# goruck/semantic-segmentation-server

Measured on AMD Instinct MI355X. Metric: frames/sec (whole node) + p50 GetSegmentedObjects latency, 513x513 PASCAL VOC, higher is better.
Workload: dtype bf16; 1 GPU; model=DeepLabv3-MobileNetV2, aspp=full, global_batch=32, per_gpu_batch=32, seq_len=513, input=513x513, camera=640x480, classes=21, parallelism=dp1, ingest=local, gather=host, backend=hip, hipgraph=True, contour_mode=fast, streams_per_gpu=1, stream_mode=batched

## Files before the change

### csrc/hip/bindings.cpp

```cpp
#include <pybind11/pybind11.h>

#include <vector>

#include "kernels.h"

namespace py = pybind11;
using namespace ssa;

namespace {
template <class T>
T* P(uintptr_t v) { return reinterpret_cast<T*>(v); }
hipStream_t S(uintptr_t v) { return reinterpret_cast<hipStream_t>(v); }
}

PYBIND11_MODULE(_hip, m) {
  m.doc() = "gfx950 HIP kernels for DeepLabv3 inference and contour statistics";

  m.def("conv_gemm",
        [](uintptr_t in, uintptr_t w, uintptr_t bias, uintptr_t img_bias, uintptr_t res,
           uintptr_t out, int B, int IH, int IW, int Cin, int OH, int OW, int Cout, int KH, int KW,
           int stride, int dil, int ldo, int co_off, int ldr, int act, uintptr_t stream, int variant,
           uintptr_t perm, int Mp) {
          ConvParams p;
          p.perm = P<const int>(perm); p.Mp = Mp;
          p.in = P<const bf16>(in); p.w = P<const bf16>(w); p.bias = P<const float>(bias);
          p.img_bias = P<const float>(img_bias); p.res = P<const bf16>(res); p.out = P<bf16>(out);
          p.B = B; p.IH = IH; p.IW = IW; p.Cin = Cin; p.OH = OH; p.OW = OW; p.Cout = Cout;
          p.KH = KH; p.KW = KW; p.stride = stride; p.dil = dil; p.ldo = ldo; p.co_off = co_off;
          p.ldr = ldr; p.act = act; p.variant = variant;
          conv_gemm(p, S(stream));
        },
        py::arg("in"), py::arg("w"), py::arg("bias"), py::arg("img_bias"), py::arg("res"),
        py::arg("out"), py::arg("B"), py::arg("IH"), py::arg("IW"), py::arg("Cin"), py::arg("OH"),
        py::arg("OW"), py::arg("Cout"), py::arg("KH"), py::arg("KW"), py::arg("stride"),
        py::arg("dil"), py::arg("ldo"), py::arg("co_off"), py::arg("ldr"), py::arg("act"),
        py::arg("stream"), py::arg("variant") = 0, py::arg("perm") = 0, py::arg("Mp") = 0);

  m.def("conv_gemm_grouped",
        [](py::list groups, uintptr_t order, int nblocks, int variant, uintptr_t stream, int ks, uintptr_t part,
           uintptr_t cnt, int cnt_stride) {
          std::vector<ConvParams> ps;
          for (auto item : groups) {
            auto t = item.cast<py::tuple>();
            if (t.size() != 23) throw std::invalid_argument("conv_gemm_grouped: 23-tuple per conv");
            auto I = [&](int i) { return t[i].cast<int>(); };
            auto U = [&](int i) { return t[i].cast<uintptr_t>(); };
            ConvParams p;
            p.in = P<const bf16>(U(0)); p.w = P<const bf16>(U(1)); p.bias = P<const float>(U(2));
            p.img_bias = P<const float>(U(3)); p.res = P<const bf16>(U(4)); p.out = P<bf16>(U(5));
            p.B = I(6); p.IH = I(7); p.IW = I(8); p.Cin = I(9); p.OH = I(10); p.OW = I(11);
            p.Cout = I(12); p.KH = I(13); p.KW = I(14); p.stride = I(15); p.dil = I(16);
            p.ldo = I(17); p.co_off = I(18); p.ldr = I(19); p.act = I(20);
            p.perm = P<const int>(U(21)); p.Mp = I(22);
            ps.push_back(p);
          }
          conv_gemm_grouped(ps.data(), (int)ps.size(), P<const int>(order), nblocks, variant,
                            S(stream), ks, P<float>(part), P<int>(cnt), cnt_stride);
        },
        py::arg("groups"), py::arg("order"), py::arg("nblocks"), py::arg("variant"),
        py::arg("stream"), py::arg("ks") = 1, py::arg("part") = 0, py::arg("cnt") = 0,
        py::arg("cnt_stride") = 0);

  m.def("bias_act", [](uintptr_t in, uintptr_t bias, uintptr_t img_bias, uintptr_t out, long long M,
                       int N, int HW, int act, uintptr_t stream) {
    bias_act(P<const bf16>(in), P<const float>(bias), P<const float>(img_bias), P<bf16>(out), M, N, HW,
             act, S(stream));
  });

  m.def("fused_ir",
        [](uintptr_t in, uintptr_t we, uintptr_t be, uintptr_t wd, uintptr_t bd, uintptr_t wp,
           uintptr_t bp, uintptr_t out, int B, int IH, int IW, int Cin, int CinP, int hidP,
           int Cout, int OH, int OW, int stride, int residual, uintptr_t stream, int dil, int TY,
           int TX, uintptr_t wd_h, uintptr_t bd_h, uintptr_t wp_h, uintptr_t trace) {
          FusedIRParams p;
          p.in = P<const bf16>(in); p.we = P<const bf16>(we); p.be = P<const float>(be);
          p.wd = P<const float>(wd); p.bd = P<const float>(bd); p.wp = P<const bf16>(wp);
          p.bp = P<const float>(bp); p.out = P<bf16>(out);
          p.B = B; p.IH = IH; p.IW = IW; p.Cin = Cin; p.CinP = CinP; p.hidP = hidP; p.Cout = Cout;
          p.OH = OH; p.OW = OW; p.stride = stride; p.residual = residual;
          p.dil = dil; p.TY = TY; p.TX = TX;
          p.wd_h = P<const void>(wd_h); p.bd_h = P<const void>(bd_h); p.wp_h = P<const void>(wp_h);
          p.trace = P<long long>(trace);
          fused_inverted_residual(p, S(stream));
        },
        py::arg("in"), py::arg("we"), py::arg("be"), py::arg("wd"), py::arg("bd"), py::arg("wp"),
        py::arg("bp"), py::arg("out"), py::arg("B"), py::arg("IH"), py::arg("IW"), py::arg("Cin"),
        py::arg("CinP"), py::arg("hidP"), py::arg("Cout"), py::arg("OH"), py::arg("OW"),
        py::arg("stride"), py::arg("residual"), py::arg("stream"), py::arg("dil") = 1,
        py::arg("TY") = 0, py::arg("TX") = 0, py::arg("wd_h") = 0, py::arg("bd_h") = 0,
        py::arg("wp_h") = 0, py::arg("trace") = 0);
  m.def("fused_ir_stream",
        [](uintptr_t in, uintptr_t w, uintptr_t bp, uintptr_t table, uintptr_t out, int B, int H,
           int W, int Cin, int hidP, int Cout, int dil, int residual, int nspan, int WR, int WCP,
           int hstride, int nh_max, uintptr_t stream, uintptr_t trace, int variant, int hsplit,
           uintptr_t part, uintptr_t cnt) {
          FusedSpanParams p;
          p.trace = P<long long>(trace);
          p.hsplit = hsplit;
          p.part = P<float>(part);
          p.cnt = P<int>(cnt);
          p.npi = variant;
          p.in = P<const bf16>(in); p.w = P<const void>(w); p.bp = P<const float>(bp);
          p.table = P<const int>(table); p.out = P<bf16>(out);
          p.B = B; p.H = H; p.W = W; p.Cin = Cin; p.hidP = hidP; p.Cout = Cout; p.dil = dil;
          p.residual = residual; p.S = nspan; p.WR = WR; p.WCP = WCP; p.hstride = hstride;
          p.nh_max = nh_max;
          fused_ir_stream(p, S(stream));
        },
        py::arg("in"), py::arg("w"), py::arg("bp"), py::arg("table"), py::arg("out"), py::arg("B"),
        py::arg("H"), py::arg("W"), py::arg("Cin"), py::arg("hidP"), py::arg("Cout"), py::arg("dil"),
        py::arg("residual"), py::arg("nspan"), py::arg("WR"), py::arg("WCP"), py::arg("hstride"),
        py::arg("nh_max"), py::arg("stream"), py::arg("trace") = 0, py::arg("variant") = 0,
        py::arg("hsplit") = 1, py::arg("part") = 0, py::arg("cnt") = 0);
  m.def("fused_ir_stream_lds", &fused_ir_stream_lds, py::arg("Cin"), py::arg("Cout"), py::arg("WR"),
        py::arg("WCP"), py::arg("nsl") = 0);
  m.def("stream_combine",
        [](uintptr_t part, uintptr_t bp, uintptr_t res, uintptr_t out, int HS, long long M, int Cout,
           uintptr_t stream, int act) {
          stream_combine(P<const float>(part), P<const float>(bp), P<const bf16>(res), P<bf16>(out), HS, M, Cout,
                         S(stream), act);
        },
        py::arg("part"), py::arg("bp"), py::arg("res"), py::arg("out"), py::arg("HS"), py::arg("M"),
        py::arg("Cout"), py::arg("stream"), py::arg("act") = 0);
  m.def("fused_ir_band",
        [](uintptr_t in, uintptr_t blob, uintptr_t out, int B, int IH, int IW, int Cin, int OH, int OW,
           int Cout, int hidP, int stride, int residual, int R, int nslot, int blob_bytes, int o_be,
           int o_wd, int o_bd, int o_wp, int o_bp, uintptr_t stream, int hs, int split) {
          FusedBandParams p;
          p.hs = hs;
          p.split = split;
          p.in = P<const bf16>(in); p.blob = P<const void>(blob); p.out = P<bf16>(out);
          p.B = B; p.IH = IH; p.IW = IW; p.Cin = Cin; p.OH = OH; p.OW = OW; p.Cout = Cout;
          p.hidP = hidP; p.stride = stride; p.residual = residual; p.R = R; p.nslot = nslot;
          p.blob_bytes = blob_bytes; p.o_be = o_be; p.o_wd = o_wd; p.o_bd = o_bd; p.o_wp = o_wp;
          p.o_bp = o_bp;
          fused_ir_band(p, S(stream));
        },
        py::arg("in"), py::arg("blob"), py::arg("out"), py::arg("B"), py::arg("IH"), py::arg("IW"),
        py::arg("Cin"), py::arg("OH"), py::arg("OW"), py::arg("Cout"), py::arg("hidP"), py::arg("stride"),
        py::arg("residual"), py::arg("R"), py::arg("nslot"), py::arg("blob_bytes"), py::arg("o_be"),
        py::arg("o_wd"), py::arg("o_bd"), py::arg("o_wp"), py::arg("o_bp"), py::arg("stream"),
        py::arg("hs") = 1, py::arg("split") = 1);
  m.def("fused_ir_slice",
        [](uintptr_t in, uintptr_t blob, uintptr_t out, int B, int IH, int IW, int Cin, int OH, int OW,
           int Cout, int hidP, int stride, int residual, int R, int o_be, int o_wd, int o_bd, int o_wp,
           int o_bp, int nw, uintptr_t stream, int one_barrier, uintptr_t lut_y, int H, int rf_s,
           int rf_a, int rf_b) {
          FusedBandParams p;
          p.lut_y = P<const int32_t>(lut_y); p.H = H; p.rf_s = rf_s; p.rf_a = rf_a; p.rf_b = rf_b;
          p.in = P<const bf16>(in); p.blob = P<const void>(blob); p.out = P<bf16>(out);
          p.B = B; p.IH = IH; p.IW = IW; p.Cin = Cin; p.OH = OH; p.OW = OW; p.Cout = Cout;
          p.hidP = hidP; p.stride = stride; p.residual = residual; p.R = R;
          p.o_be = o_be; p.o_wd = o_wd; p.o_bd = o_bd; p.o_wp = o_wp; p.o_bp = o_bp;
          fused_ir_slice(p, nw, S(stream), one_barrier != 0);
        },
        py::arg("in"), py::arg("blob"), py::arg("out"), py::arg("B"), py::arg("IH"), py::arg("IW"),
        py::arg("Cin"), py::arg("OH"), py::arg("OW"), py::arg("Cout"), py::arg("hidP"), py::arg("stride"),
        py::arg("residual"), py::arg("R"), py::arg("o_be"), py::arg("o_wd"), py::arg("o_bd"),
        py::arg("o_wp"), py::arg("o_bp"), py::arg("nw"), py::arg("stream"), py::arg("one_barrier") = 0,
        py::arg("lut_y") = 0, py::arg("H") = 0, py::arg("rf_s") = 0, py::arg("rf_a") = 0, py::arg("rf_b") = 0);
  m.def("fused_ir_slice_lds", &fused_ir_slice_lds, py::arg("stride"), py::arg("hidP"), py::arg("OW"),
        py::arg("Cout"), py::arg("nw"), py::arg("one_barrier") = false);
  m.def("fused_ir_band_lds", &fused_ir_band_lds, py::arg("stride"), py::arg("hidP"), py::arg("OW"),
        py::arg("blob_bytes"), py::arg("nslot"), py::arg("hs") = 1, py::arg("Cout") = 0,
        py::arg("split") = 1);
  m.def("fused_ir_tile_lds", &fused_ir_tile_lds);
  m.def("stem_block0",
        [](uintptr_t frames, uintptr_t lx, uintptr_t ly, uintptr_t ws, uintptr_t bs, uintptr_t wd,
           uintptr_t bd, uintptr_t wp, uintptr_t bp, uintptr_t out, int B, int Hc, int Wc, int H,
           int W, int SH, int SW, int Cout, int TY, int TX, uintptr_t stream) {
          StemBlock0Params p;
          p.frames = P<const uint8_t>(frames); p.lut_x = P<const int32_t>(lx); p.lut_y = P<const int32_t>(ly);
          p.ws = P<const bf16>(ws); p.bs = P<const float>(bs); p.wd = P<const void>(wd);
          p.bd = P<const void>(bd); p.wp = P<const void>(wp); p.bp = P<const float>(bp); p.out = P<bf16>(out);
          p.B = B; p.Hc = Hc; p.Wc = Wc; p.H = H; p.W = W; p.SH = SH; p.SW = SW; p.Cout = Cout;
          p.TY = TY; p.TX = TX;
          stem_block0(p, S(stream));
        });
  m.def("stem_band",
        [](uintptr_t frames, uintptr_t lx, uintptr_t ly, uintptr_t ws, uintptr_t bs, uintptr_t wd,
           uintptr_t bd, uintptr_t wp, uintptr_t bp, uintptr_t out, int B, int Hc, int Wc, int H,
           int W, int SH, int SW, int R, int nbx, uintptr_t stream, int one_barrier, int rf_s, int rf_a,
           int rf_b) {
          StemBlock0Params p;
          p.rf_s = rf_s; p.rf_a = rf_a; p.rf_b = rf_b;
          p.frames = P<const uint8_t>(frames); p.lut_x = P<const int32_t>(lx); p.lut_y = P<const int32_t>(ly);
          p.ws = P<const bf16>(ws); p.bs = P<const float>(bs); p.wd = P<const void>(wd);
          p.bd = P<const void>(bd); p.wp = P<const void>(wp); p.bp = P<const float>(bp); p.out = P<bf16>(out);
          p.B = B; p.Hc = Hc; p.Wc = Wc; p.H = H; p.W = W; p.SH = SH; p.SW = SW; p.Cout = 16;
          p.TY = R;
          stem_band(p, nbx, S(stream), one_barrier != 0);
        },
        py::arg("frames"), py::arg("lx"), py::arg("ly"), py::arg("ws"), py::arg("bs"), py::arg("wd"),
        py::arg("bd"), py::arg("wp"), py::arg("bp"), py::arg("out"), py::arg("B"), py::arg("Hc"),
        py::arg("Wc"), py::arg("H"), py::arg("W"), py::arg("SH"), py::arg("SW"), py::arg("R"),
        py::arg("nbx"), py::arg("stream"), py::arg("one_barrier") = 1, py::arg("rf_s") = 0,
        py::arg("rf_a") = 0, py::arg("rf_b") = 0);
  m.def("stem_band_lds", &stem_band_lds, py::arg("SW"), py::arg("nbx"), py::arg("R"));

  m.def("aspp_head",
        [](uintptr_t cat, uintptr_t wp, uintptr_t bp, uintptr_t img_bias, uintptr_t wl, uintptr_t bl,
           uintptr_t out, int M, int K, int HW, int ncls, int ldo, int G, uintptr_t stream, int waves) {
          AsppHeadParams p;
          p.waves = waves;
          p.cat = P<const bf16>(cat); p.wp = P<const bf16>(wp); p.bp = P<const float>(bp);
          p.img_bias = P<const float>(img_bias); p.wl = P<const bf16>(wl); p.bl = P<const float>(bl);
          p.out = P<bf16>(out);
          p.M = M; p.K = K; p.HW = HW; p.ncls = ncls; p.ldo = ldo; p.G = G;
          aspp_head(p, S(stream));
        },
        py::arg("cat"), py::arg("wp"), py::arg("bp"), py::arg("img_bias"), py::arg("wl"), py::arg("bl"),
        py::arg("out"), py::arg("M"), py::arg("K"), py::arg("HW"), py::arg("ncls"), py::arg("ldo"),
        py::arg("G"), py::arg("stream"), py::arg("waves") = 8);

// ... 226 lines not shown
```

### csrc/hip/conv_gemm.hip

```cpp
#include "common.h"
#include "kernels.h"

namespace ssa {

struct ConvArgs {
  const bf16* in; const bf16* w; const float* bias; const float* img_bias;
  const bf16* res; bf16* out;
  int B, IH, IW, Cin, OH, OW, Cout;
  int KH, KW, stride, dil;
  int ldo, co_off, ldr, act;
  const int* perm;
  int Mp;
};

constexpr int kMaxConvGroup = 4;
struct ConvGroupArgs {
  ConvArgs g[kMaxConvGroup];
  const int* order;
  int ks;
  float* part;
  int* cnt;
  int cnt_stride;
};

template <int MT, int NT>
__global__ __launch_bounds__(256) void conv_gemm_kernel(ConvArgs a) {
  const int lane = threadIdx.x & 63;
  const int wid = threadIdx.x >> 6;
  const int wm = wid >> 1, wn = wid & 1;
  const int M = a.B * a.OH * a.OW;
  const int tiles_m = cdiv_dev(M, 32 * MT);
  const int tiles_n = cdiv_dev(a.Cout, 32 * NT);
  const int bid = xcd_remap(blockIdx.x, tiles_m * tiles_n);
  const int tn = bid % tiles_n, tm = bid / tiles_n;
  const int pix0 = tm * 32 * MT + wm * 16 * MT;
  const int ch0 = tn * 32 * NT + wn * 16 * NT;
  const int r = lane & 15, kq = lane >> 4;

  int pb[MT], py[MT], px[MT];
  bool pvalid[MT];
#pragma unroll
  for (int i = 0; i < MT; ++i) {
    const int m = pix0 + i * 16 + r;
    pvalid[i] = m < M;
    const int mm = pvalid[i] ? m : 0;
    pb[i] = mm / (a.OH * a.OW);
    const int rem = mm - pb[i] * a.OH * a.OW;
    py[i] = (rem / a.OW) * a.stride;
    px[i] = (rem % a.OW) * a.stride;
  }
  bool wvalid[NT];
#pragma unroll
  for (int j = 0; j < NT; ++j) wvalid[j] = (ch0 + j * 16 + r) < a.Cout;

  f32x4 acc[MT][NT];
#pragma unroll
  for (int i = 0; i < MT; ++i)
#pragma unroll
    for (int j = 0; j < NT; ++j) acc[i][j] = f32x4{0.f, 0.f, 0.f, 0.f};

  const int taps = a.KH * a.KW;
  const long long wrow = (long long)taps * a.Cin;
  for (int t = 0; t < taps; ++t) {
    const int dy = (t / a.KW - a.KH / 2) * a.dil;
    const int dx = (t % a.KW - a.KW / 2) * a.dil;
    long long off[MT];
    bool ok[MT];
    bool any = false;
#pragma unroll
    for (int i = 0; i < MT; ++i) {
      const int iy = py[i] + dy, ix = px[i] + dx;
      ok[i] = pvalid[i] && iy >= 0 && iy < a.IH && ix >= 0 && ix < a.IW;
      off[i] = (((long long)pb[i] * a.IH + iy) * a.IW + ix) * a.Cin;
      any |= ok[i];
    }
    if (!__any(any)) continue;
    const bf16* wt = a.w + (long long)t * a.Cin;
    for (int c0 = 0; c0 < a.Cin; c0 += 32) {
      const int c = c0 + kq * 8;
      const bool cok = c < a.Cin;
      bf16x8 bfr[MT], afr[NT];
#pragma unroll
      for (int i = 0; i < MT; ++i)
        bfr[i] = (ok[i] && cok) ? ld8(a.in + off[i] + c) : zero8();
#pragma unroll
      for (int j = 0; j < NT; ++j)
        afr[j] = (wvalid[j] && cok) ? ld8(wt + (long long)(ch0 + j * 16 + r) * wrow + c) : zero8();
#pragma unroll
      for (int i = 0; i < MT; ++i)
#pragma unroll
        for (int j = 0; j < NT; ++j)
          acc[i][j] = __builtin_amdgcn_mfma_f32_16x16x32_bf16(afr[j], bfr[i], acc[i][j], 0, 0, 0);
    }
  }

#pragma unroll
  for (int i = 0; i < MT; ++i) {
    const int m = pix0 + i * 16 + r;
    if (m >= M) continue;
    const int b = pb[i];
#pragma unroll
    for (int j = 0; j < NT; ++j) {
      const int n = ch0 + j * 16 + kq * 4;
      if (n >= a.Cout) continue;
      float v[4] = {acc[i][j][0], acc[i][j][1], acc[i][j][2], acc[i][j][3]};
      const bool full = n + 3 < a.Cout;
#pragma unroll
      for (int q = 0; q < 4; ++q) {
        if (n + q < a.Cout) {
          v[q] += a.bias[n + q];
          if (a.img_bias) v[q] += a.img_bias[(long long)b * a.Cout + n + q];
        }
      }
      if (a.res) {
        const bf16* rp = a.res + (long long)m * a.ldr + n;
        if (full && (a.ldr & 3) == 0) {
          const bf16x4 rv = *reinterpret_cast<const bf16x4*>(rp);
#pragma unroll
          for (int q = 0; q < 4; ++q) v[q] += (float)rv[q];
        } else {
          for (int q = 0; q < 4; ++q) if (n + q < a.Cout) v[q] += (float)rp[q];
        }
      }
      bf16* op = a.out + (long long)m * a.ldo + a.co_off + n;
      if (full && ((a.ldo | a.co_off) & 3) == 0) {
        bf16x4 o;
#pragma unroll
        for (int q = 0; q < 4; ++q) o[q] = (bf16)apply_act(v[q], a.act);
        *reinterpret_cast<bf16x4*>(op) = o;
      } else {
        for (int q = 0; q < 4; ++q)
          if (n + q < a.Cout) op[q] = (bf16)apply_act(v[q], a.act);
      }
    }
  }
}

template <int MT, int NT, int KS>
__global__ __launch_bounds__(256) void conv1x1_kernel(ConvArgs a) {
  const int lane = threadIdx.x & 63, wid = threadIdx.x >> 6;
  const int wm = wid >> 1, wn = wid & 1;
  const int M = a.B * a.OH * a.OW;
  const int tiles_m = cdiv_dev(M, 32 * MT), tiles_n = cdiv_dev(a.Cout, 32 * NT);
  const int bid = xcd_remap(blockIdx.x, tiles_m * tiles_n);
  const int tn = bid % tiles_n, tm = bid / tiles_n;
  const int pix0 = tm * 32 * MT + wm * 16 * MT;
  const int ch0 = tn * 32 * NT + wn * 16 * NT;
  const int r = lane & 15, kq = lane >> 4;
  bf16x8 bfr[KS][MT], afr[KS][NT];
#pragma unroll
  for (int i = 0; i < MT; ++i) {
    const int m = pix0 + i * 16 + r;
    const bf16* src = a.in + (size_t)(m < M ? m : 0) * a.Cin + kq * 8;
#pragma unroll
    for (int k = 0; k < KS; ++k) bfr[k][i] = m < M ? ld8(src + k * 32) : zero8();
  }
#pragma unroll
  for (int j = 0; j < NT; ++j) {
    const int n = ch0 + j * 16 + r;
    const bf16* src = a.w + (size_t)(n < a.Cout ? n : 0) * a.Cin + kq * 8;
#pragma unroll
    for (int k = 0; k < KS; ++k) afr[k][j] = n < a.Cout ? ld8(src + k * 32) : zero8();
  }
  f32x4 acc[MT][NT];
#pragma unroll
  for (int i = 0; i < MT; ++i)
#pragma unroll
    for (int j = 0; j < NT; ++j) {
      f32x4 c = {0.f, 0.f, 0.f, 0.f};
#pragma unroll
      for (int k = 0; k < KS; ++k) c = __builtin_amdgcn_mfma_f32_16x16x32_bf16(afr[k][j], bfr[k][i], c, 0, 0, 0);
      acc[i][j] = c;
    }
  const int HW = a.OH * a.OW;
#pragma unroll
  for (int j = 0; j < NT; ++j) {
// ... 377 lines not shown
      for (int j = 0; j < NT; ++j) {
        const int n = wn * 16 * NT + j * 16 + r16;
        afr[j] = *reinterpret_cast<const bf16x8*>(sB + n * ROWB + ((kc ^ (n % CPR)) << 4));
      }
      __builtin_amdgcn_s_setprio(1);
#pragma unroll
      for (int i = 0; i < MT; ++i)
#pragma unroll
        for (int j = 0; j < NT; ++j)
          acc[i][j] = __builtin_amdgcn_mfma_f32_16x16x32_bf16(afr[j], bfr[i], acc[i][j], 0, 0, 0);
      __builtin_amdgcn_s_setprio(0);
    }
  }

  if (part) {
    const size_t slab = (size_t)a.B * a.OH * a.OW * a.ldo;
#pragma unroll
    for (int i = 0; i < MT; ++i) {
      const int mg = m0 + wm * 16 * MT + i * 16 + r16;
      if (mg >= M) continue;
      const int m = a.perm ? a.perm[mg] : mg;
      if (m < 0) continue;
#pragma unroll
      for (int j = 0; j < NT; ++j) {
        const int n = n0 + wn * 16 * NT + j * 16 + kq * 4;
        if (n < a.Cout) *reinterpret_cast<f32x4*>(part + kslice * slab + (size_t)m * a.ldo + a.co_off + n) = acc[i][j];
      }
    }
    if (cnt) {
      asm volatile("s_waitcnt vmcnt(0)" ::: "memory");
      __syncthreads();
      int* s_flag = reinterpret_cast<int*>(smem);
      if (tid == 0) {
        __builtin_amdgcn_fence(__ATOMIC_RELEASE, "agent");
        asm volatile("s_waitcnt vmcnt(0)" ::: "memory");
        const int t = __hip_atomic_fetch_add(cnt + bid, 1, __ATOMIC_RELAXED, __HIP_MEMORY_SCOPE_AGENT);
        const int last = t == ks - 1;
        if (last) {
          __hip_atomic_store(cnt + bid, 0, __ATOMIC_RELAXED, __HIP_MEMORY_SCOPE_AGENT);
          __builtin_amdgcn_fence(__ATOMIC_ACQUIRE, "agent");
          asm volatile("s_waitcnt vmcnt(0)" ::: "memory");
        }
        *s_flag = last;
      }
      __syncthreads();
      if (*reinterpret_cast<volatile int*>(s_flag)) {
        constexpr int NTH = 64 * NW, Q = BN / 4;
        for (int idx = tid; idx < BM * Q; idx += NTH) {
          const int r = idx / Q, n = n0 + (idx - r * Q) * 4;
          const int mg = m0 + r;
          if (mg >= M || n >= a.Cout) continue;
          const int m = a.perm ? a.perm[mg] : mg;
          if (m < 0) continue;
          const float* q = part + (size_t)m * a.ldo + a.co_off + n;
          f32x4 v = *reinterpret_cast<const f32x4*>(a.bias + n);
          for (int s0 = 0; s0 < ks; s0 += kInlineKS) {
            f32x4 pv[kInlineKS];
#pragma unroll
            for (int sl = 0; sl < kInlineKS; ++sl)
              pv[sl] = *reinterpret_cast<const f32x4*>(q + (size_t)(s0 + sl < ks ? s0 + sl : ks - 1) * slab);
#pragma unroll
            for (int sl = 0; sl < kInlineKS; ++sl)
              if (s0 + sl < ks) v += pv[sl];
          }
          bf16x4 o;
#pragma unroll
          for (int e = 0; e < 4; ++e) o[e] = (bf16)apply_act(v[e], a.act);
          *reinterpret_cast<bf16x4*>(a.out + (size_t)m * a.ldo + a.co_off + n) = o;
        }
      }
    }
    return;
  }
  f32x4 bj[NT];
#pragma unroll
  for (int j = 0; j < NT; ++j) {
    const int n = n0 + wn * 16 * NT + j * 16 + kq * 4;
    if (n + 3 < a.Cout) {
      bj[j] = *reinterpret_cast<const f32x4*>(a.bias + n);
    } else {
#pragma unroll
      for (int q = 0; q < 4; ++q) bj[j][q] = n + q < a.Cout ? a.bias[n + q] : 0.f;
    }
  }
#pragma unroll
  for (int i = 0; i < MT; ++i) {
    const int mg = m0 + wm * 16 * MT + i * 16 + r16;
    if (mg >= M) continue;
    const int m = a.perm ? a.perm[mg] : mg;
    if (m < 0) continue;
#pragma unroll
    for (int j = 0; j < NT; ++j) {
      const int n = n0 + wn * 16 * NT + j * 16 + kq * 4;
      if (n >= a.Cout) continue;
      float v[4] = {acc[i][j][0] + bj[j][0], acc[i][j][1] + bj[j][1], acc[i][j][2] + bj[j][2],
                    acc[i][j][3] + bj[j][3]};
      const bool full = n + 3 < a.Cout;
      if (a.img_bias) {
        const int b = m / (a.OH * a.OW);
#pragma unroll
        for (int q = 0; q < 4; ++q)
          if (n + q < a.Cout) v[q] += a.img_bias[(long long)b * a.Cout + n + q];
      }
      if (a.res) {
        const bf16* rp = a.res + (long long)m * a.ldr + n;
        if (full && (a.ldr & 3) == 0) {
          const bf16x4 rv4 = *reinterpret_cast<const bf16x4*>(rp);
#pragma unroll
          for (int q = 0; q < 4; ++q) v[q] += (float)rv4[q];
        } else {
          for (int q = 0; q < 4; ++q) if (n + q < a.Cout) v[q] += (float)rp[q];
        }
      }
      bf16* op = a.out + (long long)m * a.ldo + a.co_off + n;
      if (full && ((a.ldo | a.co_off) & 3) == 0) {
        bf16x4 o;
#pragma unroll
        for (int q = 0; q < 4; ++q) o[q] = (bf16)apply_act(v[q], a.act);
        *reinterpret_cast<bf16x4*>(op) = o;
      } else {
        for (int q = 0; q < 4; ++q)
          if (n + q < a.Cout) op[q] = (bf16)apply_act(v[q], a.act);
      }
    }
  }
}

template <int MT, int NT, int ST, int WM = 2, int WN = 2>
__global__ __launch_bounds__(64 * WM * WN) void conv_glds_kernel(ConvArgs a) {
  extern __shared__ __attribute__((aligned(16))) char smem[];
  constexpr int BM = 16 * MT * WM, BN = 16 * NT * WN;
  const int M = a.perm ? a.Mp : a.B * a.OH * a.OW;
  const int tiles = cdiv_dev(M, BM) * cdiv_dev(a.Cout, BN);
  glds_tile<MT, NT, ST, WM, WN>(a, xcd_remap(blockIdx.x, tiles), smem);
}

template <int MT, int NT, int ST, int WM = 2, int WN = 2, int BK = 64>
__global__ __launch_bounds__(64 * WM * WN) void conv_glds_group_kernel(ConvGroupArgs ga) {
  extern __shared__ __attribute__((aligned(16))) char smem[];
  const int e = __builtin_amdgcn_readfirstlane(ga.order[blockIdx.x]);
  const int t = e & 0xfffff, ksl = (e >> 20) & 15;
  switch (e >> 24) {
    case 0: glds_tile<MT, NT, ST, WM, WN, BK>(ga.g[0], t, smem, ga.ks, ksl, ga.part, ga.cnt); break;
    case 1: glds_tile<MT, NT, ST, WM, WN, BK>(ga.g[1], t, smem, ga.ks, ksl, ga.part,
                                              ga.cnt ? ga.cnt + ga.cnt_stride : nullptr); break;
    case 2: glds_tile<MT, NT, ST, WM, WN, BK>(ga.g[2], t, smem, ga.ks, ksl, ga.part,
                                              ga.cnt ? ga.cnt + 2 * ga.cnt_stride : nullptr); break;
    default: glds_tile<MT, NT, ST, WM, WN, BK>(ga.g[3], t, smem, ga.ks, ksl, ga.part,
                                               ga.cnt ? ga.cnt + 3 * ga.cnt_stride : nullptr); break;
  }
}

template <int MT, int NT, int ST, int WM = 2, int WN = 2, int BK = 64>
static void launch_conv_glds_group(const ConvGroupArgs& ga, int nblocks, hipStream_t s) {
  constexpr int BM = 16 * MT * WM, BN = 16 * NT * WN;
  const size_t lds = (size_t)ST * (BM + BN) * BK * 2 + 16;
  static_assert((size_t)ST * (BM + BN) * BK * 2 + 16 <= 160 * 1024, "LDS ring too large");
  static bool attr_set = false;
  if (!attr_set) {
    check(hipFuncSetAttribute(reinterpret_cast<const void*>(&conv_glds_group_kernel<MT, NT, ST, WM, WN, BK>),
                              hipFuncAttributeMaxDynamicSharedMemorySize, 160 * 1024),
          "conv_glds_group attr");
    attr_set = true;
  }
  hipLaunchKernelGGL((conv_glds_group_kernel<MT, NT, ST, WM, WN, BK>), dim3(nblocks),
                     dim3(64 * WM * WN), lds, s, ga);
  check_launch("conv_glds_group");
}

template <int MT, int NT, int ST, int WM = 2, int WN = 2>
static void launch_conv_glds(const ConvArgs& a, hipStream_t s) {
  constexpr int BM = 16 * MT * WM, BN = 16 * NT * WN;
  const int M = a.perm ? a.Mp : a.B * a.OH * a.OW;
  const int grid = cdiv(M, BM) * cdiv(a.Cout, BN);
  const size_t lds = (size_t)ST * (BM + BN) * 128 + 16;
  static bool attr_set = false;
  if (!attr_set) {
    check(hipFuncSetAttribute(reinterpret_cast<const void*>(&conv_glds_kernel<MT, NT, ST, WM, WN>),
                              hipFuncAttributeMaxDynamicSharedMemorySize, 160 * 1024),
          "conv_glds attr");
    attr_set = true;
  }
  hipLaunchKernelGGL((conv_glds_kernel<MT, NT, ST, WM, WN>), dim3(grid), dim3(64 * WM * WN), lds, s, a);
  check_launch("conv_glds");
}

template <int ST>
static void dispatch_glds(const ConvArgs& a, hipStream_t s) {
  switch (pick_nt(a.Cout)) {
    case 1: launch_conv_glds<4, 1, ST>(a, s); break;
    case 2: launch_conv_glds<4, 2, ST>(a, s); break;
    case 3: launch_conv_glds<4, 3, ST>(a, s); break;
    case 4: launch_conv_glds<4, 4, ST>(a, s); break;
    case 5: launch_conv_glds<4, 5, ST>(a, s); break;
    default: launch_conv_glds<4, 6, ST>(a, s); break;
  }
}

template <int MT, int NT, int KS>
static void launch_conv_lds(const ConvArgs& a, hipStream_t s) {
  const int M = a.B * a.OH * a.OW;
  const int grid = cdiv(M, 32 * MT) * cdiv(a.Cout, 32 * NT);
  const size_t lds = (size_t)2 * (32 * MT + 32 * NT) * 32 * KS * sizeof(bf16) + 16;
  hipLaunchKernelGGL((conv_gemm_lds_kernel<MT, NT, KS>), dim3(grid), dim3(256), lds, s, a);
  check_launch("conv_gemm_lds");
}

static int pick_nt(int Cout) {
  if (Cout <= 192) return (Cout + 31) / 32;
  int best = 4, waste = 1 << 30;
  for (int nt = 6; nt >= 4; --nt) {
    const int w = cdiv(Cout, 32 * nt) * 32 * nt - Cout;
    if (w < waste) { waste = w; best = nt; }
  }
  return best;
}

template <int KS>
static void dispatch_lds(const ConvArgs& a, hipStream_t s) {
  switch (pick_nt(a.Cout)) {
    case 1: launch_conv_lds<4, 1, KS>(a, s); break;
    case 2: launch_conv_lds<4, 2, KS>(a, s); break;
    case 3: launch_conv_lds<4, 3, KS>(a, s); break;
    case 4: launch_conv_lds<4, 4, KS>(a, s); break;
    case 5: launch_conv_lds<4, 5, KS>(a, s); break;
    default: launch_conv_lds<4, 6, KS>(a, s); break;
  }
}

template <int MT, int NT>
static void launch_conv(const ConvArgs& a, hipStream_t s) {
  const int M = a.B * a.OH * a.OW;
  const int grid = cdiv(M, 32 * MT) * cdiv(a.Cout, 32 * NT);
  hipLaunchKernelGGL((conv_gemm_kernel<MT, NT>), dim3(grid), dim3(256), 0, s, a);
  check_launch("conv_gemm");
}

void conv_gemm(const ConvParams& p, hipStream_t s) {
  if (p.Cin % 8 != 0) throw std::invalid_argument("conv_gemm: Cin must be a multiple of 8");
  if (p.co_off % 1 != 0 || p.ldo < p.co_off + p.Cout) throw std::invalid_argument("conv_gemm: bad ldo/co_off");
  if (p.res && p.ldr < p.Cout) throw std::invalid_argument("conv_gemm: bad ldr");
  ConvArgs a{p.in, p.w, p.bias, p.img_bias, p.res, p.out, p.B, p.IH, p.IW, p.Cin, p.OH, p.OW,
             p.Cout, p.KH, p.KW, p.stride, p.dil, p.ldo, p.co_off, p.ldr, p.act, p.perm, p.Mp};
  const long long M = (long long)p.B * p.OH * p.OW;
  const long long tiles = (M + 127) / 128 * cdiv(p.Cout, 32 * pick_nt(p.Cout));
  const long long K = (long long)p.KH * p.KW * p.Cin;
  const bool glds_ok = (long long)p.B * p.IH * p.IW * p.Cin < (1LL << 30) &&
                       (long long)p.Cout * K < (1LL << 30) && p.KH * p.KW <= 16;
  int variant = p.variant;
  if (variant == 0) variant = (tiles >= 128 && K >= 256) ? (glds_ok ? 4 : 2) : 1;
  if (p.perm && (variant < 3 || variant == 7 || variant > 10 || !glds_ok))
    throw std::invalid_argument("conv_gemm: a pixel permutation needs an LDS-DMA variant (3-6)");
  if (variant == 3 || variant == 4) {
    if (!glds_ok) throw std::invalid_argument("conv_gemm glds: tensor too large for 32-bit offsets or > 16 taps");
    if (variant == 3) dispatch_glds<3>(a, s);
    else dispatch_glds<2>(a, s);
    return;
  }
  if (variant >= 8 && variant <= 10) {
    if (!glds_ok) throw std::invalid_argument("conv_gemm glds: tensor too large for 32-bit offsets or > 16 taps");
    if (variant == 8) launch_conv_glds<4, 4, 3, 2, 4>(a, s);
    else if (variant == 10) launch_conv_glds<4, 4, 4, 2, 2>(a, s);
    else switch (pick_nt(p.Cout)) {
      case 1: launch_conv_glds<2, 1, 4, 2, 2>(a, s); break;
      case 2: launch_conv_glds<2, 2, 4, 2, 2>(a, s); break;
      case 3: launch_conv_glds<2, 3, 4, 2, 2>(a, s); break;
      case 4: launch_conv_glds<2, 4, 4, 2, 2>(a, s); break;
      case 5: launch_conv_glds<2, 5, 4, 2, 2>(a, s); break;
      default: launch_conv_glds<2, 6, 4, 2, 2>(a, s); break;
    }
    return;
  }
  if (variant == 5 || variant == 6) {
    if (!glds_ok) throw std::invalid_argument("conv_gemm glds: tensor too large for 32-bit offsets or > 16 taps");
    if (variant == 5) launch_conv_glds<4, 4, 2, 2, 4>(a, s);
    else launch_conv_glds<8, 4, 2, 2, 4>(a, s);
    return;
  }
  if (variant == 2) {
    if (p.Cin <= 32) dispatch_lds<1>(a, s);
    else dispatch_lds<2>(a, s);
    return;
  }
  const bool k1 = p.KH == 1 && p.KW == 1 && p.stride == 1 && p.OH == p.IH && p.OW == p.IW &&
                  p.Cin % 32 == 0 && p.Cin <= 192 && M * (long long)p.Cin < (1LL << 31);
  if (k1 && (variant == 7 || p.variant == 0)) {
    bool ok;
    if (p.Cout <= 32) ok = launch_conv1x1<4, 1>(a, s);
    else if (p.Cout <= 64 || M < 8192) ok = launch_conv1x1<2, 2>(a, s);
    else ok = launch_conv1x1<2, 4>(a, s);
    if (ok) return;
  }
  if (p.Cout <= 32) {
    launch_conv<4, 1>(a, s);
  } else if (p.Cout <= 64 || M < 8192) {
    launch_conv<2, 2>(a, s);
  } else {
    launch_conv<2, 4>(a, s);
  }
}

static ConvArgs to_args(const ConvParams& p) {
  return ConvArgs{p.in, p.w, p.bias, p.img_bias, p.res, p.out, p.B, p.IH, p.IW, p.Cin, p.OH, p.OW,
                  p.Cout, p.KH, p.KW, p.stride, p.dil, p.ldo, p.co_off, p.ldr, p.act, p.perm, p.Mp};
}

void conv_gemm_grouped(const ConvParams* ps, int n, const int* order, int nblocks, int variant,
                       hipStream_t s, int ks, float* part, int* cnt, int cnt_stride) {
  if (n < 1 || n > kMaxConvGroup) throw std::invalid_argument("conv_gemm_grouped: 1..4 convs");
  if (!order || nblocks < 1) throw std::invalid_argument("conv_gemm_grouped: empty tile order");
  if (ks < 1 || ks > 16 || (ks > 1 && part == nullptr))
    throw std::invalid_argument("conv_gemm_grouped: ks in [1, 16], a partials buffer for ks > 1");
  if (ks > 1)
    for (int i = 0; i < n; ++i)
      if (ps[i].ldo != ps[0].ldo || ps[i].Cout % 4 || (ps[i].ldo | ps[i].co_off) % 4)
        throw std::invalid_argument("conv_gemm_grouped: split-K needs one ldo and 4-aligned channels");
  ConvGroupArgs ga{};
  ga.ks = ks;
  ga.part = ks > 1 ? part : nullptr;
  ga.cnt = ks > 1 ? cnt : nullptr;
  ga.cnt_stride = cnt_stride;
  for (int i = 0; i < kMaxConvGroup; ++i) {
    const ConvParams& p = ps[i < n ? i : 0];
    if (p.Cin % 8 != 0 || p.KH * p.KW > 16 || p.Cout != ps[0].Cout)
      throw std::invalid_argument("conv_gemm_grouped: Cin % 8, <= 16 taps and one Cout required");
    if ((long long)p.B * p.IH * p.IW * p.Cin >= (1LL << 30) ||
        (long long)p.Cout * p.KH * p.KW * p.Cin >= (1LL << 30))
      throw std::invalid_argument("conv_gemm_grouped: tensor too large for 32-bit byte offsets");
    ga.g[i] = to_args(p);
  }
  ga.order = order;
  switch (variant) {
    case 5: launch_conv_glds_group<4, 4, 2, 2, 4>(ga, nblocks, s); break;
    case 6: launch_conv_glds_group<8, 4, 2, 2, 4>(ga, nblocks, s); break;
    case 8: launch_conv_glds_group<4, 4, 3, 2, 4>(ga, nblocks, s); break;
    case 10: launch_conv_glds_group<4, 4, 4, 2, 2>(ga, nblocks, s); break;
    case 11: launch_conv_glds_group<4, 4, 2, 2, 2>(ga, nblocks, s); break;
    case 12: launch_conv_glds_group<8, 4, 4, 2, 4, 32>(ga, nblocks, s); break;
    case 13: launch_conv_glds_group<4, 4, 4, 2, 4, 32>(ga, nblocks, s); break;
    case 14: launch_conv_glds_group<8, 4, 3, 2, 4, 32>(ga, nblocks, s); break;
    case 15: launch_conv_glds_group<4, 4, 2, 4, 4>(ga, nblocks, s); break;
    case 16: launch_conv_glds_group<4, 4, 4, 4, 4, 32>(ga, nblocks, s); break;
    case 17: launch_conv_glds_group<2, 4, 2, 4, 4>(ga, nblocks, s); break;
    case 18: launch_conv_glds_group<4, 2, 2, 4, 4>(ga, nblocks, s); break;
    default: throw std::invalid_argument("conv_gemm_grouped: variant must be 5, 6, 8, 10-18");
  }
}

}
```

### csrc/hip/kernels.h

```cpp
#pragma once
#include <hip/hip_runtime.h>
#include <stdint.h>

#include "common.h"

namespace ssa {

struct ConvParams {
  const bf16* in = nullptr;
  const bf16* w = nullptr;
  const float* bias = nullptr;
  const float* img_bias = nullptr;
  const bf16* res = nullptr;
  bf16* out = nullptr;
  int B = 0, IH = 0, IW = 0, Cin = 0, OH = 0, OW = 0, Cout = 0;
  int KH = 1, KW = 1, stride = 1, dil = 1;
  int ldo = 0, co_off = 0, ldr = 0, act = 0;
  int variant = 0;
  const int* perm = nullptr;
  int Mp = 0;
};
void conv_gemm(const ConvParams& p, hipStream_t s);
void conv_gemm_grouped(const ConvParams* ps, int n, const int* order, int nblocks, int variant,
                       hipStream_t s, int ks = 1, float* part = nullptr, int* cnt = nullptr,
                       int cnt_stride = 0);

struct PwConvParams {
  const bf16* in = nullptr;
  const bf16* w = nullptr;
  const float* img_bias = nullptr;
  const bf16* res = nullptr;
  bf16* out = nullptr;
  int M = 0, K = 0, N = 0, HW = 1, ldo = 0, co_off = 0, ldr = 0, act = 0;
  int mt = 2;
  int nch = 1;
  int out_f16 = 0;
};
void pw_conv(const PwConvParams& p, hipStream_t s);

struct TapConvParams {
  const bf16* in = nullptr;
  const bf16* w = nullptr;
  const float* bias = nullptr;
  bf16* out = nullptr;
  const int* perm = nullptr;
  int Mp = 0;
  int B = 0, H = 0, W = 0, Cin = 0, Cout = 0, KH = 3, KW = 3, dil = 1, ldo = 0, co_off = 0, act = 0;
};
void tap_conv(const TapConvParams& p, hipStream_t s);
int tap_conv_group_channels();
int pw_conv_supported_ks(int K);

struct ConvI8Params {
  const int8_t* in = nullptr;
  const int8_t* w = nullptr;
  const float* scale = nullptr;
  const float* bias = nullptr;
  const float* img_bias = nullptr;
  const int8_t* res = nullptr;
  float res_scale = 0.f;
  void* out = nullptr;
  float inv_out_scale = 1.f;
  int out_mode = 0;
  int B = 0, IH = 0, IW = 0, Cin = 0, OH = 0, OW = 0, Cout = 0;
  int KH = 1, KW = 1, stride = 1, dil = 1, ldo = 0, co_off = 0, act = 0;
  int variant = 0;
  const int* perm = nullptr;
  int Mp = 0;
};
void conv_i8(const ConvI8Params& p, hipStream_t s);
void conv_i8_grouped(const ConvI8Params* ps, int n, const int* order, int nblocks, int variant,
                     hipStream_t s);
void maxpool3x3s2_i8(const int8_t* in, int8_t* out, int B, int IH, int IW, int C, int OH, int OW,
                     hipStream_t s);
void global_avgpool_i8(const int8_t* in, float* out, float* ws, int B, int HW, int C, float scale,
                       hipStream_t s);

struct FusedIRParams {
  const bf16* in = nullptr;
  const bf16* we = nullptr;
  const float* be = nullptr;
  const float* wd = nullptr;
  const float* bd = nullptr;
  const bf16* wp = nullptr;
  const float* bp = nullptr;
  bf16* out = nullptr;
  int B = 0, IH = 0, IW = 0, Cin = 0, CinP = 0, hidP = 0, Cout = 0, OH = 0, OW = 0;
  int stride = 1, residual = 0;
  int dil = 1;
  int TY = 0, TX = 0;
  const void* wd_h = nullptr;
  const void* bd_h = nullptr;
  const void* wp_h = nullptr;
  long long* trace = nullptr;
};
void fused_inverted_residual(const FusedIRParams& p, hipStream_t s);
struct FusedSpanParams {
  const bf16* in = nullptr;
  const void* w = nullptr;
  const float* bp = nullptr;
  const int* table = nullptr;
  bf16* out = nullptr;
  int B = 0, H = 0, W = 0, Cin = 0, hidP = 0, Cout = 0, dil = 1, residual = 0;
  int S = 8, WR = 0, WCP = 0, hstride = 0;
  int npi = 0;
  long long* trace = nullptr;
  int nh_max = 0;
  int hsplit = 1;
  float* part = nullptr;
  int* cnt = nullptr;
};
void fused_ir_stream(const FusedSpanParams& p, hipStream_t s);
size_t fused_ir_stream_lds(int Cin, int Cout, int WR, int WCP, int nsl = 0);
void stream_combine(const float* part, const float* bp, const bf16* res, bf16* out, int HS, long long M, int Cout,
                    hipStream_t st, int act = 0);
struct FusedBandParams {
  const bf16* in = nullptr;
  const void* blob = nullptr;
  bf16* out = nullptr;
  int B = 0, IH = 0, IW = 0, Cin = 0, OH = 0, OW = 0, Cout = 0, hidP = 0, stride = 1, residual = 0;
  int R = 8, nslot = 2, blob_bytes = 0, o_be = 0, o_wd = 0, o_bd = 0, o_wp = 0, o_bp = 0;
  int hs = 1;
  int split = 1;
  const int32_t* lut_y = nullptr;
  int H = 0, rf_s = 0, rf_a = 0, rf_b = 0;
};
void fused_ir_band(const FusedBandParams& p, hipStream_t s);
size_t fused_ir_band_lds(int stride, int hidP, int OW, int blob_bytes, int nslot, int hs = 1, int Cout = 0,
                         int split = 1);
int fused_ir_band_cols(int stride);
void fused_ir_slice(const FusedBandParams& p, int nw, hipStream_t s, bool one_barrier = false);
size_t fused_ir_slice_lds(int stride, int hidP, int OW, int Cout, int nw, bool one_barrier = false);
struct StemBlock0Params {
  const uint8_t* frames = nullptr; const int32_t* lut_x = nullptr; const int32_t* lut_y = nullptr;
  const bf16* ws = nullptr; const float* bs = nullptr;
  const void* wd = nullptr; const void* bd = nullptr; const void* wp = nullptr;
  const float* bp = nullptr; bf16* out = nullptr;
  int B = 0, Hc = 0, Wc = 0, H = 0, W = 0, SH = 0, SW = 0, Cout = 16, TY = 8, TX = 16;
  int rf_s = 0, rf_a = 0, rf_b = 0;
};
void stem_block0(const StemBlock0Params& p, hipStream_t s);
void stem_band(const StemBlock0Params& p, int nbx, hipStream_t s, bool one_barrier = true);
size_t stem_band_lds(int SW, int nbx, int R);
size_t fused_ir_tile_lds(int CinP, int stride, int dil, int TY, int TX, int expand);

struct AsppHeadParams {
  const bf16* cat = nullptr;
  const bf16* wp = nullptr;
  const float* bp = nullptr;
  const float* img_bias = nullptr;
  const bf16* wl = nullptr;
  const float* bl = nullptr;
  bf16* out = nullptr;
  int M = 0, K = 0, N = 256, HW = 0, ncls = 0, ldo = 0;
  int G = 9;
  int waves = 8;
};
void aspp_head(const AsppHeadParams& p, hipStream_t s);
size_t aspp_head_lds(int G, int K);

struct DwProjectParams {
  const bf16* hid_in = nullptr;
  const float* wd = nullptr;
  const float* bd = nullptr;
  const bf16* wp = nullptr;
  const float* bp = nullptr;
  const bf16* res = nullptr;
  bf16* out = nullptr;
  int B = 0, IH = 0, IW = 0, hid = 0, Cout = 0, OH = 0, OW = 0, stride = 1, dil = 1;
};
void dw_project(const DwProjectParams& p, hipStream_t s);

struct DwProjFusedParams {
  const void* h = nullptr;
  const void* w = nullptr;
  const float* bp = nullptr;
  const bf16* res = nullptr;
  bf16* out = nullptr;
// ... 70 lines not shown
```

### csrc/hip/model_ops.hip

```cpp
#include "common.h"
#include "kernels.h"

namespace ssa {

__global__ __launch_bounds__(256) void dw3x3_kernel(const bf16* __restrict__ in,
                                                    const float* __restrict__ w,
                                                    const float* __restrict__ bias,
                                                    bf16* __restrict__ out, int B, int IH, int IW,
                                                    int C, int OH, int OW, int stride, int dil,
                                                    int act) {
  const int CG = C >> 3;
  const long long total = (long long)B * OH * OW * CG;
  for (long long t = (long long)blockIdx.x * blockDim.x + threadIdx.x; t < total;
       t += (long long)gridDim.x * blockDim.x) {
    const int cg = (int)(t % CG);
    long long pix = t / CG;
    const int ox = (int)(pix % OW);
    pix /= OW;
    const int oy = (int)(pix % OH);
    const int b = (int)(pix / OH);
    const int c = cg * 8;
    float acc[8];
#pragma unroll
    for (int q = 0; q < 8; ++q) acc[q] = bias[c + q];
#pragma unroll
    for (int ky = 0; ky < 3; ++ky) {
      const int iy = oy * stride + (ky - 1) * dil;
      if (iy < 0 || iy >= IH) continue;
#pragma unroll
      for (int kx = 0; kx < 3; ++kx) {
        const int ix = ox * stride + (kx - 1) * dil;
        if (ix < 0 || ix >= IW) continue;
        const bf16x8 v = ld8(in + (((long long)b * IH + iy) * IW + ix) * C + c);
        const float4 w0 = *reinterpret_cast<const float4*>(w + (ky * 3 + kx) * C + c);
        const float4 w1 = *reinterpret_cast<const float4*>(w + (ky * 3 + kx) * C + c + 4);
        acc[0] += (float)v[0] * w0.x; acc[1] += (float)v[1] * w0.y;
        acc[2] += (float)v[2] * w0.z; acc[3] += (float)v[3] * w0.w;
        acc[4] += (float)v[4] * w1.x; acc[5] += (float)v[5] * w1.y;
        acc[6] += (float)v[6] * w1.z; acc[7] += (float)v[7] * w1.w;
      }
    }
    bf16x8 o;
#pragma unroll
    for (int q = 0; q < 8; ++q) o[q] = (bf16)apply_act(acc[q], act);
    st8(out + t * 8, o);
  }
}

template <int S, int D, int PX>
__global__ __launch_bounds__(256) void dw3x3_strip_kernel(const bf16* __restrict__ in,
                                                          const float* __restrict__ w,
                                                          const float* __restrict__ bias,
                                                          bf16* __restrict__ out, int B, int IH,
                                                          int IW, int C, int OH, int OW, int act) {
  constexpr int NC = (PX - 1) * S + 2 * D + 1;
  const int CG = C >> 3;
  const int SX = (OW + PX - 1) / PX;
  const int total = B * OH * SX * CG;
  const int t = blockIdx.x * blockDim.x + threadIdx.x;
  if (t >= total) return;
  const int cg = t % CG;
  int r = t / CG;
  const int sx = r % SX;
  r /= SX;
  const int oy = r % OH, b = r / OH;
  const int c = cg * 8, ox0 = sx * PX;
  float acc[PX][8];
  {
    const float4 b0 = *reinterpret_cast<const float4*>(bias + c);
    const float4 b1 = *reinterpret_cast<const float4*>(bias + c + 4);
#pragma unroll
    for (int p = 0; p < PX; ++p) {
      acc[p][0] = b0.x; acc[p][1] = b0.y; acc[p][2] = b0.z; acc[p][3] = b0.w;
      acc[p][4] = b1.x; acc[p][5] = b1.y; acc[p][6] = b1.z; acc[p][7] = b1.w;
    }
  }
#pragma unroll
  for (int ky = 0; ky < 3; ++ky) {
    const int iy = oy * S + (ky - 1) * D;
    if (iy < 0 || iy >= IH) continue;
    const bf16* row = in + ((size_t)(b * IH + iy) * IW) * C + c;
    bf16x8 col[NC];
#pragma unroll
    for (int j = 0; j < NC; ++j) {
      const int ix = ox0 * S - D + j;
      col[j] = (ix >= 0 && ix < IW) ? ld8(row + (size_t)ix * C) : zero8();
    }
#pragma unroll
    for (int kx = 0; kx < 3; ++kx) {
      const float4 w0 = *reinterpret_cast<const float4*>(w + (ky * 3 + kx) * C + c);
      const float4 w1 = *reinterpret_cast<const float4*>(w + (ky * 3 + kx) * C + c + 4);
      const float wv[8] = {w0.x, w0.y, w0.z, w0.w, w1.x, w1.y, w1.z, w1.w};
#pragma unroll
      for (int p = 0; p < PX; ++p) {
        const bf16x8 v = col[p * S + kx * D];
#pragma unroll
        for (int q = 0; q < 8; ++q) acc[p][q] += (float)v[q] * wv[q];
      }
    }
  }
  bf16* op = out + ((size_t)(b * OH + oy) * OW + ox0) * C + c;
#pragma unroll
  for (int p = 0; p < PX; ++p) {
    if (ox0 + p >= OW) break;
    bf16x8 o;
#pragma unroll
    for (int q = 0; q < 8; ++q) o[q] = (bf16)apply_act(acc[p][q], act);
    st8(op + (size_t)p * C, o);
  }
}

void depthwise3x3(const bf16* in, const float* w, const float* bias, bf16* out, int B, int IH,
                  int IW, int C, int OH, int OW, int stride, int dil, int act, hipStream_t s) {
  if (C % 8) throw std::invalid_argument("depthwise3x3: C must be a multiple of 8");
  constexpr int PX = 4;
  const long long strip_total = (long long)B * OH * ((OW + PX - 1) / PX) * (C / 8);
  if (strip_total < (1LL << 31) && (long long)B * IH * IW * C < (1LL << 40)) {
    const int grid = cdiv(strip_total, 256);
#define DWS(S_, D_)                                                                              \
    if (stride == S_ && dil == D_) {                                                             \
      hipLaunchKernelGGL((dw3x3_strip_kernel<S_, D_, PX>), dim3(grid), dim3(256), 0, s, in, w,   \
                         bias, out, B, IH, IW, C, OH, OW, act);                                  \
      check_launch("depthwise3x3 strip");                                                        \
      return;                                                                                    \
    }
    DWS(1, 1) DWS(1, 2) DWS(2, 1) DWS(1, 4)
#undef DWS
  }
  const long long total = (long long)B * OH * OW * (C / 8);
  const int grid = (int)std::min<long long>(cdiv(total, 256), 256LL * 32);
  hipLaunchKernelGGL(dw3x3_kernel, dim3(grid), dim3(256), 0, s, in, w, bias, out, B, IH, IW, C,
                     OH, OW, stride, dil, act);
  check_launch("depthwise3x3");
}

template <int COUT>
__global__ __launch_bounds__(256) void stem_kernel(const uint8_t* __restrict__ frames,
                                                   const int32_t* __restrict__ lut_x,
                                                   const int32_t* __restrict__ lut_y,
                                                   const float* __restrict__ w,
                                                   const float* __restrict__ bias,
                                                   void* __restrict__ outv, int B, int Hc, int Wc,
                                                   int H, int W, int OH, int OW, int K,
                                                   int stride, int act, float out_inv_scale) {
  extern __shared__ __attribute__((aligned(16))) float sw[];
  const int nw = K * K * 3 * COUT;
  for (int i = threadIdx.x; i < nw; i += blockDim.x) sw[i] = w[i];
  for (int i = threadIdx.x; i < COUT; i += blockDim.x) sw[nw + i] = bias[i];
  __syncthreads();
  const long long total = (long long)B * OH * OW;
  const long long t = (long long)blockIdx.x * blockDim.x + threadIdx.x;
  if (t >= total) return;
// ... 150 lines not shown
#pragma unroll
        for (int q = 0; q < 4; ++q) o[q] = (bf16)apply_act(acc[q], a.act);
        *reinterpret_cast<bf16x4*>(static_cast<bf16*>(a.out) + pix * Cout + n) = o;
      }
    }
  }
}

template <int KG>
__global__ __launch_bounds__(256) void stem_mfma_ws_kernel(SMArgs a) {
  extern __shared__ __attribute__((aligned(16))) char smem[];
  bf16* IN = reinterpret_cast<bf16*>(smem);
  const int IHT = (a.TY - 1) * a.stride + a.K, IWT = (a.TX - 1) * a.stride + a.K;
  const int ntile = a.tiles_y * a.tiles_x;
  const int bid = xcd_remap(blockIdx.x, gridDim.x);
  const int b = bid / ntile, t = bid % ntile;
  const int oy0 = (t / a.tiles_x) * a.TY, ox0 = (t % a.tiles_x) * a.TX;
  const int iy0 = oy0 * a.stride - a.K / 2, ix0 = ox0 * a.stride - a.K / 2;
  const int tid = threadIdx.x, lane = tid & 63;
  const int sub = __builtin_amdgcn_readfirstlane(tid >> 6);
  const int r16 = lane & 15, kq = lane >> 4;
  const float inv_tx = 1.f / a.TX;
  const uint8_t* fb = a.frames + (size_t)b * a.Hc * a.Wc * 3;
  gather_letterbox_rgb0<6, 256>(IN, fb, a.lut_x, a.lut_y, a.Wc, a.H, a.W, iy0, ix0, IHT, IWT, tid);
  s16x4m wf[KG];
#pragma unroll
  for (int m = 0; m < KG; ++m)
    wf[m] = *reinterpret_cast<const s16x4m*>(a.w + (size_t)(sub * 16 + r16) * (KG * 16) + m * 16 + kq * 4);
  const f32x4 bs = *reinterpret_cast<const f32x4*>(a.bias + sub * 16 + kq * 4);
  int toff[KG];
#pragma unroll
  for (int m = 0; m < KG; ++m) {
    const int tp = m * 4 + kq;
    toff[m] = tp < a.K * a.K ? ((tp / a.K) * IWT + tp % a.K) * 4 : 0;
  }
  __syncthreads();
  const int Cout = 64;
  const int n = sub * 16 + kq * 4;
  const int groups = (a.TY * a.TX + 15) / 16;
#pragma unroll 2
  for (int g = 0; g < groups; ++g) {
    const int p = g * 16 + r16;
    const int py = (int)(((float)p + 0.5f) * inv_tx), px = p - py * a.TX;
    const int oy = oy0 + py, ox = ox0 + px;
    const bool valid = p < a.TY * a.TX && oy < a.OH && ox < a.OW;
    const int base = valid ? (py * a.stride * IWT + px * a.stride) * 4 : 0;
    s16x4m xf[KG];
#pragma unroll
    for (int m = 0; m < KG; ++m) xf[m] = *reinterpret_cast<const s16x4m*>(IN + base + toff[m]);
    f32x4 acc = bs;
#pragma unroll
    for (int m = 0; m < KG; ++m) acc = __builtin_amdgcn_mfma_f32_16x16x16bf16_1k(wf[m], xf[m], acc, 0, 0, 0);
    if (!valid) continue;
    const size_t pix = ((size_t)b * a.OH + oy) * a.OW + ox;
    if (a.out_inv_scale > 0.f && a.act == ACT_RELU) {
      unsigned w = 0;
#pragma unroll
      for (int q = 0; q < 4; ++q)
        w = __builtin_amdgcn_cvt_pk_u8_f32(__builtin_amdgcn_fmed3f(acc[q] * a.out_inv_scale, 0.f, 127.f), q, w);
      *reinterpret_cast<unsigned*>(static_cast<int8_t*>(a.out) + pix * Cout + n) = w;
    } else if (a.out_inv_scale > 0.f) {
      char4 o;
      o.x = (signed char)fminf(fmaxf(rintf(apply_act(acc[0], a.act) * a.out_inv_scale), -127.f), 127.f);
      o.y = (signed char)fminf(fmaxf(rintf(apply_act(acc[1], a.act) * a.out_inv_scale), -127.f), 127.f);
      o.z = (signed char)fminf(fmaxf(rintf(apply_act(acc[2], a.act) * a.out_inv_scale), -127.f), 127.f);
      o.w = (signed char)fminf(fmaxf(rintf(apply_act(acc[3], a.act) * a.out_inv_scale), -127.f), 127.f);
      *reinterpret_cast<char4*>(static_cast<int8_t*>(a.out) + pix * Cout + n) = o;
    } else {
      bf16x4 o;
#pragma unroll
      for (int q = 0; q < 4; ++q) o[q] = (bf16)apply_act(acc[q], a.act);
      *reinterpret_cast<bf16x4*>(static_cast<bf16*>(a.out) + pix * Cout + n) = o;
    }
  }
}

void stem_mfma(const uint8_t* frames, const int32_t* lut_x, const int32_t* lut_y, const bf16* w,
               const float* bias, void* out, int B, int Hc, int Wc, int H, int W, int OH, int OW,
               int Cout, int K, int stride, int act, float out_inv_scale, int TY, int TX,
               hipStream_t s, int mode) {
  if (mode == 1) {
    if (Cout != 64 || (K * K + 3) / 4 != 13) throw std::invalid_argument("stem_mfma ws: (Cout, K) must be (64, 7)");
    if (TY < 1 || TX < 1 || TY * TX > 1024) throw std::invalid_argument("stem_mfma ws: bad tile");
    const size_t lds = (size_t)((TY - 1) * stride + K) * ((TX - 1) * stride + K) * 8;
    if (lds > 64 * 1024) throw std::invalid_argument("stem_mfma ws: tile too large");
    SMArgs a{frames, lut_x, lut_y, w, bias, out, B, Hc, Wc, H, W, OH, OW, K, stride, act, TY, TX,
             cdiv(OH, TY), cdiv(OW, TX), out_inv_scale};
    hipLaunchKernelGGL((stem_mfma_ws_kernel<13>), dim3(B * a.tiles_y * a.tiles_x), dim3(256), lds, s, a);
    check_launch("stem_mfma ws");
    return;
  }
  if (mode != 0) throw std::invalid_argument("stem_mfma: mode must be 0 or 1");
  if (TY < 1 || TX < 1 || TY * TX > 256 || TX > 120) throw std::invalid_argument("stem_mfma: bad tile");
  const int IHT = (TY - 1) * stride + K, IWT = (TX - 1) * stride + K;
  const size_t lds = (size_t)IHT * IWT * 8;
  if (lds > 64 * 1024) throw std::invalid_argument("stem_mfma: tile too large");
  SMArgs a{frames, lut_x, lut_y, w, bias, out, B, Hc, Wc, H, W, OH, OW, K, stride, act, TY, TX,
           cdiv(OH, TY), cdiv(OW, TX), out_inv_scale};
  const int grid = B * a.tiles_y * a.tiles_x;
  const int groups = (TY * TX + 15) / 16;
  const int kg = (K * K + 3) / 4;
#define SM(NS, KGV, G) hipLaunchKernelGGL((stem_mfma_kernel<NS, KGV, G>), dim3(grid), dim3(256), lds, s, a)
  if (Cout == 64 && kg == 13) {
    if (groups <= 4) SM(4, 13, 1); else if (groups <= 8) SM(4, 13, 2); else SM(4, 13, 4);
  } else if (Cout == 32 && kg == 3) {
    if (groups <= 4) SM(2, 3, 1); else if (groups <= 8) SM(2, 3, 2); else SM(2, 3, 4);
  } else {
    throw std::invalid_argument("stem_mfma: (Cout, K) must be (64, 7) or (32, 3)");
  }
#undef SM
  check_launch("stem_mfma");
}

__global__ void maxpool_kernel(const bf16* __restrict__ in, bf16* __restrict__ out, int B, int IH,
                               int IW, int C, int OH, int OW) {
  const int CG = C >> 3;
  const long long total = (long long)B * OH * OW * CG;
  const long long t = (long long)blockIdx.x * blockDim.x + threadIdx.x;
  if (t >= total) return;
  const int cg = (int)(t % CG);
  long long pix = t / CG;
  const int ox = (int)(pix % OW);
  pix /= OW;
  const int oy = (int)(pix % OH);
  const int b = (int)(pix / OH);
  float m[8];
#pragma unroll
  for (int q = 0; q < 8; ++q) m[q] = -3.0e38f;
  for (int ky = 0; ky < 3; ++ky) {
    const int iy = oy * 2 + ky - 1;
    if (iy < 0 || iy >= IH) continue;
    for (int kx = 0; kx < 3; ++kx) {
      const int ix = ox * 2 + kx - 1;
      if (ix < 0 || ix >= IW) continue;
      const bf16x8 v = ld8(in + (((long long)b * IH + iy) * IW + ix) * C + cg * 8);
#pragma unroll
      for (int q = 0; q < 8; ++q) m[q] = fmaxf(m[q], (float)v[q]);
    }
  }
  bf16x8 o;
#pragma unroll
  for (int q = 0; q < 8; ++q) o[q] = (bf16)m[q];
  st8(out + t * 8, o);
}

void maxpool3x3s2(const bf16* in, bf16* out, int B, int IH, int IW, int C, int OH, int OW,
                  hipStream_t s) {
  const long long total = (long long)B * OH * OW * (C / 8);
  hipLaunchKernelGGL(maxpool_kernel, dim3(cdiv(total, 256)), dim3(256), 0, s, in, out, B, IH, IW,
                     C, OH, OW);
  check_launch("maxpool3x3s2");
}

constexpr int kGapSlices = 32;

__global__ __launch_bounds__(256) void gap_partial_kernel(const bf16* __restrict__ in,
                                                          float* __restrict__ part, int HW, int C) {
  const int b = blockIdx.x, sl = blockIdx.y;
  const int CG = C >> 3;
  const int lane = threadIdx.x & 63, wid = threadIdx.x >> 6;
  const int cg = blockIdx.z * 64 + lane;
  __shared__ float red[4][64][8];
  float acc[8] = {0, 0, 0, 0, 0, 0, 0, 0};
  const int p0 = (int)((long long)HW * sl / kGapSlices), p1 = (int)((long long)HW * (sl + 1) / kGapSlices);
  if (cg < CG) {
    const bf16* base = in + (long long)b * HW * C + cg * 8;
    int p = p0 + wid;
    for (; p + 12 < p1; p += 16) {
      bf16x8 v[4];
#pragma unroll
      for (int u = 0; u < 4; ++u) v[u] = ld8(base + (long long)(p + 4 * u) * C);
#pragma unroll
      for (int u = 0; u < 4; ++u)
#pragma unroll
        for (int q = 0; q < 8; ++q) acc[q] += (float)v[u][q];
    }
    for (; p < p1; p += 4) {
      const bf16x8 v = ld8(base + (long long)p * C);
#pragma unroll
      for (int q = 0; q < 8; ++q) acc[q] += (float)v[q];
    }
  }
#pragma unroll
  for (int q = 0; q < 8; ++q) red[wid][lane][q] = acc[q];
  __syncthreads();
  if (wid == 0 && cg < CG) {
#pragma unroll
    for (int q = 0; q < 8; ++q)
      part[((long long)b * kGapSlices + sl) * C + cg * 8 + q] =
          red[0][lane][q] + red[1][lane][q] + red[2][lane][q] + red[3][lane][q];
  }
}

__global__ void gap_reduce_kernel(const float* __restrict__ part, float* __restrict__ out, int B,
                                  int HW, int C) {
  const int i = blockIdx.x * blockDim.x + threadIdx.x;
  if (i >= B * C) return;
  const int b = i / C, c = i % C;
  float s = 0.f;
#pragma unroll
  for (int k = 0; k < kGapSlices; ++k) s += part[((long long)b * kGapSlices + k) * C + c];
  out[i] = s / (float)HW;
}

size_t gap_workspace_floats(int B, int C) { return (size_t)B * kGapSlices * C; }

__global__ __launch_bounds__(256) void copy_to_host_kernel(const uint4* __restrict__ src,
                                                           uint4* __restrict__ dst, long long n16,
                                                           const uint32_t* __restrict__ src4,
                                                           uint32_t* __restrict__ dst4, long long n4) {
  const long long i = (long long)blockIdx.x * blockDim.x + threadIdx.x;
  const long long stride = (long long)gridDim.x * blockDim.x;
  for (long long k = i; k < n16; k += stride) dst[k] = src[k];
  for (long long k = i; k < n4; k += stride) dst4[k] = src4[k];
}

void copy_to_host(const void* src, void* dst, long long nbytes, hipStream_t s) {
  if (nbytes % 4) throw std::invalid_argument("copy_to_host: nbytes % 4 == 0 required");
  const bool al = ((uintptr_t)src % 16 == 0) && ((uintptr_t)dst % 16 == 0);
  const long long n16 = al ? nbytes / 16 : 0;
  const long long tail = nbytes - n16 * 16;
  const auto* s4 = reinterpret_cast<const uint32_t*>(static_cast<const char*>(src) + n16 * 16);
  auto* d4 = reinterpret_cast<uint32_t*>(static_cast<char*>(dst) + n16 * 16);
  const long long work = n16 > tail / 4 ? n16 : tail / 4;
  const int grid = (int)std::min<long long>(64, std::max<long long>(1, cdiv(work, 256)));
  hipLaunchKernelGGL(copy_to_host_kernel, dim3(grid), dim3(256), 0, s, static_cast<const uint4*>(src),
                     static_cast<uint4*>(dst), n16, s4, d4, tail / 4);
  check_launch("copy_to_host");
}

__global__ __launch_bounds__(256) void pack_rows_kernel(uint32_t* __restrict__ dst,
                                                        const uint32_t* __restrict__ a, int aw,
                                                        const uint32_t* __restrict__ b, int bw,
                                                        int rows) {
  const int w = aw + bw;
  const long long n = (long long)rows * w;
  for (long long i = (long long)blockIdx.x * blockDim.x + threadIdx.x; i < n;
       i += (long long)gridDim.x * blockDim.x) {
    const long long r = i / w;
    const int c = (int)(i - r * w);
    dst[i] = c < aw ? a[r * aw + c] : b[r * bw + (c - aw)];
  }
}

void pack_rows(void* dst, const void* a, int a_words, const void* b, int b_words, int rows,
               hipStream_t s) {
  if (rows <= 0 || a_words < 0 || b_words < 0) throw std::invalid_argument("pack_rows: bad shape");
  const long long n = (long long)rows * (a_words + b_words);
  const int grid = (int)std::min<long long>(64, std::max<long long>(1, cdiv(n, 256)));
  hipLaunchKernelGGL(pack_rows_kernel, dim3(grid), dim3(256), 0, s, static_cast<uint32_t*>(dst),
                     static_cast<const uint32_t*>(a), a_words, static_cast<const uint32_t*>(b),
                     b_words, rows);
  check_launch("pack_rows");
}

void global_avgpool(const bf16* in, float* out, float* ws, int B, int HW, int C, hipStream_t s) {
  hipLaunchKernelGGL(gap_partial_kernel, dim3(B, kGapSlices, cdiv(C / 8, 64)), dim3(256), 0, s, in,
                     ws, HW, C);
  hipLaunchKernelGGL(gap_reduce_kernel, dim3(cdiv((long long)B * C, 256)), dim3(256), 0, s, ws, out,
                     B, HW, C);
  check_launch("global_avgpool");
}

__global__ __launch_bounds__(256) void matvec_kernel(const float* __restrict__ x,
                                                     const float* __restrict__ w,
                                                     const float* __restrict__ bias,
                                                     float* __restrict__ out, int B, int N, int K,
                                                     int act) {
  const int lane = threadIdx.x & 63;
  const long long item = (long long)blockIdx.x * 4 + (threadIdx.x >> 6);
  if (item >= (long long)B * N) return;
  const int b = (int)(item / N), n = (int)(item % N);
  float s = 0.f;
  for (int k = lane; k < K; k += 64) s += w[(long long)n * K + k] * x[(long long)b * K + k];
#pragma unroll
  for (int o = 32; o > 0; o >>= 1) s += __shfl_xor(s, o, 64);
  if (lane == 0) out[item] = apply_act(s + (bias ? bias[n] : 0.f), act);
}

__global__ __launch_bounds__(256) void bias_act_kernel(const bf16* __restrict__ in,
                                                       const float* __restrict__ bias,
                                                       const float* __restrict__ img_bias,
                                                       bf16* __restrict__ out, int M, int N,
                                                       int HW, int act) {
  const int NG = N >> 3;
  const int t = blockIdx.x * blockDim.x + threadIdx.x;
  if (t >= M * NG) return;
  const int m = t / NG;
  const int n = (t - m * NG) * 8;
  const bf16x8 v = ld8(in + (size_t)m * N + n);
  float4 b0 = *reinterpret_cast<const float4*>(bias + n), b1 = *reinterpret_cast<const float4*>(bias + n + 4);
  if (img_bias) {
    const float* ib = img_bias + (size_t)(m / HW) * N + n;
    const float4 i0 = *reinterpret_cast<const float4*>(ib), i1 = *reinterpret_cast<const float4*>(ib + 4);
    b0.x += i0.x; b0.y += i0.y; b0.z += i0.z; b0.w += i0.w;
    b1.x += i1.x; b1.y += i1.y; b1.z += i1.z; b1.w += i1.w;
  }
  const float bb[8] = {b0.x, b0.y, b0.z, b0.w, b1.x, b1.y, b1.z, b1.w};
  bf16x8 o;
#pragma unroll
  for (int q = 0; q < 8; ++q) o[q] = (bf16)apply_act((float)v[q] + bb[q], act);
  st8(out + (size_t)m * N + n, o);
}

void bias_act(const bf16* in, const float* bias, const float* img_bias, bf16* out, long long M, int N,
              int HW, int act, hipStream_t s) {
  if (N % 8 || HW < 1) throw std::invalid_argument("bias_act: N % 8 == 0 and HW >= 1 required");
  if (M * (long long)N >= (1LL << 31)) throw std::invalid_argument("bias_act: matrix too large");
  hipLaunchKernelGGL(bias_act_kernel, dim3(cdiv(M * (N / 8), 256)), dim3(256), 0, s, in, bias, img_bias,
                     out, (int)M, N, HW, act);
  check_launch("bias_act");
}

void matvec(const float* x, const float* w, const float* bias, float* out, int B, int N, int K,
            int act, hipStream_t s) {
  hipLaunchKernelGGL(matvec_kernel, dim3(cdiv((long long)B * N, 4)), dim3(256), 0, s, x, w, bias,
                     out, B, N, K, act);
  check_launch("matvec");
}

constexpr int kPoolMaxC = 2048, kPoolMaxN = 512;

__device__ __forceinline__ float4 pool_slice(const float* __restrict__ wt, const float* s_x, int k0,
                                             int k1, int N, int q) {
  float4 a0 = make_float4(0.f, 0.f, 0.f, 0.f), a1 = a0;
  int k = k0;
  for (; k + 2 <= k1; k += 2) {
    const float4 w0 = *reinterpret_cast<const float4*>(wt + (size_t)k * N + 4 * q);
    const float4 w1 = *reinterpret_cast<const float4*>(wt + (size_t)(k + 1) * N + 4 * q);
    const float x0 = s_x[k], x1 = s_x[k + 1];
    a0.x += w0.x * x0; a0.y += w0.y * x0; a0.z += w0.z * x0; a0.w += w0.w * x0;
    a1.x += w1.x * x1; a1.y += w1.y * x1; a1.z += w1.z * x1; a1.w += w1.w * x1;
  }
  if (k < k1) {
    const float4 w0 = *reinterpret_cast<const float4*>(wt + (size_t)k * N + 4 * q);
    const float x0 = s_x[k];
    a0.x += w0.x * x0; a0.y += w0.y * x0; a0.z += w0.z * x0; a0.w += w0.w * x0;
  }
  return make_float4(a0.x + a1.x, a0.y + a1.y, a0.z + a1.z, a0.w + a1.w);
}

template <int kPoolThreads>
__global__ __launch_bounds__(kPoolThreads) void aspp_pool_kernel(const float* __restrict__ part,
                                                                 const float* __restrict__ w1t,
                                                                 const float* __restrict__ b1,
                                                                 const float* __restrict__ w2t,
                                                                 float* __restrict__ img_bias, int HW,
                                                                 int C, int N, float* dbg, int mode) {
  __shared__ float s_gap[kPoolMaxC];
  if (mode & 1) __builtin_amdgcn_fence(__ATOMIC_ACQUIRE, "agent");
  __shared__ float s_pool[kPoolMaxN];
  __shared__ float4 s_red[kPoolThreads];
  const int b = blockIdx.x, tid = threadIdx.x;
  const float inv = 1.f / (float)HW;
  const float* pb = part + (size_t)b * kGapSlices * C;
  for (int k = tid; k < C; k += kPoolThreads) {
    float s = 0.f;
#pragma unroll
    for (int q = 0; q < kGapSlices; ++q) s += pb[(size_t)q * C + k];
    s_gap[k] = s * inv;
  }
  const int nq = N >> 2;
  const int nks = kPoolThreads / nq;
  const int q = tid % nq, ks = tid / nq;
  __syncthreads();
  const size_t dstride = (size_t)C + N + 4 * 4 * kPoolThreads;
  float* dimg = dbg ? dbg + (size_t)b * dstride : nullptr;
  float4* dv = dbg ? reinterpret_cast<float4*>(dimg + C + N) : nullptr;
  if (dbg)
    for (int k = tid; k < C; k += kPoolThreads) dimg[k] = s_gap[k];
  {
    const int per = (C + nks - 1) / nks;
    const int k0 = min(C, ks * per), k1 = min(C, k0 + per);
    if (ks < nks) {
      const float4 r = pool_slice(w1t, s_gap, k0, k1, N, q);
      s_red[ks * nq + q] = r;
      if (dbg) dv[tid] = r;
    }
  }
  __syncthreads();
  if (tid < nq) {
    float4 s = s_red[tid];
    if (dbg) dv[kPoolThreads + tid] = s;
    for (int j = 1; j < nks; ++j) {
      const float4 v = s_red[j * nq + tid];
      if (dbg) dv[kPoolThreads + j * nq + tid] = v;
      s.x += v.x; s.y += v.y; s.z += v.z; s.w += v.w;
    }
    s_pool[4 * tid + 0] = fmaxf(s.x + b1[4 * tid + 0], 0.f);
    s_pool[4 * tid + 1] = fmaxf(s.y + b1[4 * tid + 1], 0.f);
    s_pool[4 * tid + 2] = fmaxf(s.z + b1[4 * tid + 2], 0.f);
    s_pool[4 * tid + 3] = fmaxf(s.w + b1[4 * tid + 3], 0.f);
  }
  __syncthreads();
  if (dbg)
    for (int k = tid; k < N; k += kPoolThreads) dimg[C + k] = s_pool[k];
  {
    const int per = (N + nks - 1) / nks;
    const int k0 = min(N, ks * per), k1 = min(N, k0 + per);
    if (ks < nks) {
      const float4 r = pool_slice(w2t, s_pool, k0, k1, N, q);
      s_red[ks * nq + q] = r;
      if (dbg) dv[2 * kPoolThreads + tid] = r;
    }
  }
  __syncthreads();
  if (tid < nq) {
    float4 s = s_red[tid];
    if (dbg) dv[3 * kPoolThreads + tid] = s;
    for (int j = 1; j < nks; ++j) {
      const float4 v = s_red[j * nq + tid];
      if (dbg) dv[3 * kPoolThreads + j * nq + tid] = v;
      s.x += v.x; s.y += v.y; s.z += v.z; s.w += v.w;
    }
    *reinterpret_cast<float4*>(img_bias + (size_t)b * N + 4 * tid) = s;
  }
}

void aspp_pool(const bf16* in, float* ws, const float* w1t, const float* b1, const float* w2t,
               float* img_bias, int B, int HW, int C, int N, hipStream_t s, float* dbg, int mode) {
  if (C > kPoolMaxC || N > kPoolMaxN || C % 8 || N % 4)
    throw std::invalid_argument("aspp_pool: C <= 2048, C % 8, N <= 512, N % 4");
  if (!(mode & 2))
    hipLaunchKernelGGL(gap_partial_kernel, dim3(B, kGapSlices, cdiv(C / 8, 64)), dim3(256), 0, s, in,
                       ws, HW, C);
  if (mode & 4)
    hipLaunchKernelGGL(aspp_pool_kernel<256>, dim3(B), dim3(256), 0, s, ws, w1t, b1, w2t, img_bias, HW, C,
                       N, dbg, mode);
  else if (mode & 8)
    hipLaunchKernelGGL(aspp_pool_kernel<512>, dim3(B), dim3(512), 0, s, ws, w1t, b1, w2t, img_bias, HW, C,
                       N, dbg, mode);
  else
    hipLaunchKernelGGL(aspp_pool_kernel<1024>, dim3(B), dim3(1024), 0, s, ws, w1t, b1, w2t, img_bias, HW,
                       C, N, dbg, mode);
  check_launch("aspp_pool");
}

template <int KMAX>
__global__ __launch_bounds__(256) void upsample_argmax_kernel(const bf16* __restrict__ logits,
                                                              uint8_t* __restrict__ labels, int B,
                                                              int h, int w, int K, int ldk, int H,
                                                              int W) {
  const int W4 = (W + 3) / 4;
  const long long total = (long long)B * H * W4;
  const long long t = (long long)blockIdx.x * blockDim.x + threadIdx.x;
  if (t >= total) return;
  const int xq = (int)(t % W4);
  const int Y = (int)((t / W4) % H);
  const int b = (int)(t / ((long long)W4 * H));
  const float sh = H > 1 ? (float)(h - 1) / (float)(H - 1) : 0.f;
  const float sw = W > 1 ? (float)(w - 1) / (float)(W - 1) : 0.f;
  const float fy = sh * (float)Y;
  const int y0 = (int)fy;
  const int yp = y0 < h - 1 ? 1 : 0;
  const float ly1 = fy - (float)y0, ly0 = 1.f - ly1;
  const bf16* L = logits + (long long)b * h * w * ldk;
  uint32_t packed = 0;
  for (int e = 0; e < 4; ++e) {
    const int X = xq * 4 + e;
    if (X >= W) break;
    const float fx = sw * (float)X;
    const int x0 = (int)fx;
    const int xp = x0 < w - 1 ? 1 : 0;
    const float lx1 = fx - (float)x0, lx0 = 1.f - lx1;
    const bf16* p00 = L + ((long long)y0 * w + x0) * ldk;
    const bf16* p01 = p00 + xp * ldk;
    const bf16* p10 = p00 + (long long)yp * w * ldk;
    const bf16* p11 = p10 + xp * ldk;
    float best = -3.0e38f;
    int arg = 0;
#pragma unroll 4
    for (int k = 0; k < K; ++k) {
      const float v = ly0 * (lx0 * (float)p00[k] + lx1 * (float)p01[k]) +
                      ly1 * (lx0 * (float)p10[k] + lx1 * (float)p11[k]);
      if (v > best) { best = v; arg = k; }
    }
    packed |= (uint32_t)(arg & 0xff) << (8 * e);
  }
  uint8_t* op = labels + ((long long)b * H + Y) * W + xq * 4;
  if (xq * 4 + 3 < W && ((((uintptr_t)op) & 3) == 0)) {
    *reinterpret_cast<uint32_t*>(op) = packed;
  } else {
    for (int e = 0; e < 4 && xq * 4 + e < W; ++e) op[e] = (packed >> (8 * e)) & 0xff;
  }
}

__device__ __forceinline__ int wave_max_int(int v) {
#pragma unroll
  for (int off = 1; off < 64; off <<= 1) v = max(v, __shfl_xor(v, off));
  return v;
}

template <int KP, int KC = 0>
struct Interval {
  static constexpr int NK = KC ? KC : KP;
  float v0[KP], dv[KP];
  int xs, xe;
  float sw;
  int j, w;

  __device__ void load(const bf16* __restrict__ logits, int b, int Y, int jj, int h, int ww, int H,
                       int W, int ldk) {
    j = jj;
    w = ww;
    const float sh = H > 1 ? (float)(h - 1) / (float)(H - 1) : 0.f;
    sw = W > 1 ? (float)(w - 1) / (float)(W - 1) : 0.f;
    const float fy = sh * (float)Y;
    const int y0 = (int)fy;
    const int yp = y0 < h - 1 ? 1 : 0;
    const float ly1 = fy - (float)y0, ly0 = 1.f - ly1;
    xs = sw > 0.f ? (int)((float)j / sw) - 1 : 0;
    if (xs < 0) xs = 0;
    while (xs > 0 && (int)(sw * (float)xs) >= j) --xs;
    while (xs < W && (int)(sw * (float)xs) < j) ++xs;
    xe = xs;
    for (int e = 0; e < 32; ++e) {
      const int X = xs + e;
      if (X >= W || (int)(sw * (float)X) != j) break;
      xe = X + 1;
    }
    const int j1 = j < w - 1 ? j + 1 : j;
    const bf16* r0 = logits + ((size_t)(b * h + y0) * w) * ldk;
    const bf16* r1 = r0 + (size_t)yp * w * ldk;
#pragma unroll
    for (int k8 = 0; k8 < KP; k8 += 8) {
      const bf16x8 a0 = ld8(r0 + (size_t)j * ldk + k8), a1 = ld8(r1 + (size_t)j * ldk + k8);
      const bf16x8 c0 = ld8(r0 + (size_t)j1 * ldk + k8), c1 = ld8(r1 + (size_t)j1 * ldk + k8);
#pragma unroll
      for (int q = 0; q < 8; ++q) {
        if (k8 + q >= NK) continue;
        const float u = ly0 * (float)a0[q] + ly1 * (float)a1[q];
        const float v = ly0 * (float)c0[q] + ly1 * (float)c1[q];
        v0[k8 + q] = u;
        dv[k8 + q] = v - u;
      }
    }
  }

  __device__ float lx(int X) const { return j < w - 1 ? sw * (float)X - (float)j : 0.f; }

  template <bool TAGGED>
  __device__ int argmax_at(float lx1, int K) const {
    float best = -3.0e38f;
    int arg = 0;
#pragma unroll
    for (int k = 0; k < NK; ++k) {
      const float v = v0[k] + lx1 * dv[k];
      if (TAGGED) {
        const float t = __uint_as_float((__float_as_uint(v) & ~31u) | (unsigned)(31 - k));
        if (KC || k < K) best = fmaxf(best, t);
      } else {
        if ((KC || k < K) && v > best) { best = v; arg = k; }
      }
    }
    return TAGGED ? 31 - (int)(__float_as_uint(best) & 31u) : arg;
  }

  template <int NPX>
  __device__ void emit_union(uint8_t* op, int K) const {
    const int n = xe - xs;
    const float t0 = lx(xs), t1 = lx(n > 0 ? xe - 1 : xs);
    float hi[KP];
    float L = -3.0e38f, M = 0.f;
#pragma unroll
    for (int k = 0; k < NK; ++k) {
      const float a = v0[k] + t0 * dv[k], b = v0[k] + t1 * dv[k];
      const float lo = fminf(a, b);
      hi[k] = fmaxf(a, b);
      if (KC || k < K) {
// ... 264 lines not shown
```

### semantic_segmentation_server_amd/models/hip_model.py

```python
from __future__ import annotations

import os
from types import SimpleNamespace
from typing import Callable, Dict, List, Optional, Tuple

import torch

from ..ops import fused_band as FB
from ..ops import fused_span as FS
from ..ops import hip_ops as K
from ..ops import row_repeat as RR
from ..ops.hip_ops import conv_out_hw
from .deeplab import DeepLabV3
from .layers import ConvBNAct
from .mobilenetv2 import MobileNetV2Backbone
from .plan import TUNE_FILE_DEFAULT, Choice, HipPlanModel


def _pack_dense(layer: ConvBNAct, dev) -> Tuple[torch.Tensor, torch.Tensor]:
    w, b = layer.fold()
    return (w.permute(0, 2, 3, 1).contiguous().to(dev, torch.bfloat16),
            b.contiguous().to(dev, torch.float32))


def _pack_dw(layer: ConvBNAct, dev) -> Tuple[torch.Tensor, torch.Tensor]:
    w, b = layer.fold()
    return (w.reshape(w.shape[0], 9).t().contiguous().to(dev, torch.float32),
            b.contiguous().to(dev, torch.float32))


def _pack_stem(layer: ConvBNAct, dev) -> Tuple[torch.Tensor, torch.Tensor]:
    w, b = layer.fold()
    return (w.permute(2, 3, 1, 0).reshape(-1, w.shape[0]).contiguous().to(dev, torch.float32),
            b.contiguous().to(dev, torch.float32))


def _fold_block(m) -> tuple:
    ew = eb = None
    if m.expand is not None:
        ew, eb = m.expand.fold()
        ew = ew[:, :, 0, 0]
    dwf, dbf = m.dw.fold()
    pwf, pbf = m.project.fold()
    return ew, eb, dwf[:, 0], dbf, pwf[:, :, 0, 0], pbf


_TILES = [(8, 16), (4, 16), (11, 11), (5, 11), (8, 13), (5, 13), (16, 16), (11, 22)]


def _tile_candidates(OH: int, OW: int, CinP: int, stride: int, dil: int,
                     expand: bool = True) -> List[Tuple[int, int]]:
    out = []
    for ty, tx in _TILES:
        if -(-ty * tx // 16) > 8 or K.fused_ir_tile_lds(CinP, stride, dil, ty, tx, expand) > 160 * 1024:
            continue
        covered = -(-OH // ty) * ty * -(-OW // tx) * tx
        if covered <= 1.25 * OH * OW:
            out.append((ty, tx))
    return out


_PW_CONFIGS = [(2, 1), (2, 2), (2, 3), (4, 3), (4, 5)]


def pw_choice(name: str, gemm_op: Callable, x: torch.Tensor, w: torch.Tensor, b: torch.Tensor,
              out: torch.Tensor, *, M: int, Cin: int, Cout: int, ldo: Optional[int] = None,
              co_off: int = 0, act=None, N_out: Optional[int] = None) -> Callable:
    Np = max(Cout, N_out or Cout)
    if not K.pw_supported(Cin, Np) or (ldo or Np) % 8 or co_off % 8:
        return gemm_op
    wpk = K.pack_pw_weights(w, b, N_out=Np)
    variants = [("gemm", [gemm_op])]
    NC = -(-Np // 64)
    for mt, nch in _PW_CONFIGS:
        if nch > NC:
            continue
        variants.append((f"pw{mt}x{nch}", [
            lambda *_, mt=mt, nch=nch: K.pw_conv(x, wpk, out, M=M, K=Cin, N=Np, ldo=ldo,
                                                  co_off=co_off, act=act, mt=mt, nch=nch)]))
    return Choice(name, variants)


def _dwp_rows_fit(ty: int, stages: int, dil: int, OW: int, cout: int) -> bool:
    nw = -(-ty * OW // 16)
    if nw > 16:
        return False
    halo = -(-(ty + 2 * dil) * (OW + 2 * dil) // 64) * 64
    return (halo // 16 <= 4 * nw and
            stages * (halo * 64 + (cout // 16 + 1) * 1024) <= 160 * 1024)


def _rows_per_band(work: int, OH: int, targets) -> List[int]:
    return list(dict.fromkeys(min(max(2, -(-work // target)), OH) for target in targets))


class HipDeepLab(HipPlanModel):
    def __init__(self, model: DeepLabV3, device: torch.device, cfg=None):
        super().__init__(model, device, cfg.input_size if cfg is not None else 513)
        dev = device
        bb = model.backbone
        self.kind = "mnv2" if isinstance(bb, MobileNetV2Backbone) else "resnet50"
        self.stem = _pack_stem(bb.stem, dev) + (bb.stem.k, bb.stem.stride, bb.stem.act, bb.stem.cout)
        self.blocks: List[dict] = []
        self.stem_block0 = None
        if self.kind == "mnv2":
            self.blocks = [self._pack_mnv2_block(blk, dev) for blk in bb.blocks]
            b0 = bb.blocks[0]
            s0 = b0.spec
            if (b0.expand is None and s0.stride == 1 and s0.dilation == 1 and s0.cin == 32 and
                    s0.cout == 16 and bb.stem.cout == 32 and bb.stem.k == 3 and bb.stem.stride == 2
                    and bb.stem.act == "relu6"):
                self.stem_block0 = K.pack_stem_block0(bb.stem, *_fold_block(b0)[2:], dev)
        else:
            for blk in bb.blocks:
                self.blocks.append(dict(
                    blk=blk,
                    conv1=_pack_dense(blk.conv1, dev), conv2=_pack_dense(blk.conv2, dev),
                    conv3=_pack_dense(blk.conv3, dev),
                    down=_pack_dense(blk.down, dev) if blk.down is not None else None))
        aspp = model.aspp
        self.aspp_c = aspp.cout
        self.aspp_b0 = _pack_dense(aspp.b0, dev)
        self.aspp_atrous = [(_pack_dense(b, dev), b.dilation) for b in aspp.atrous]
        self.cat_c = (1 + len(aspp.atrous)) * aspp.cout
        pw, pb = aspp.project.fold()
        pw = pw[:, :, 0, 0]
        self.proj_w = pw[:, : self.cat_c].contiguous().to(dev, torch.bfloat16)
        self.proj_b = pb.to(dev, torch.float32)
        self.has_pool = aspp.pool is not None
        if self.has_pool:
            qw, qb = aspp.pool.fold()
            self.pool_w = qw[:, :, 0, 0].contiguous().to(dev, torch.float32)
            self.pool_b = qb.to(dev, torch.float32)
            self.proj_pool_w = pw[:, self.cat_c:].contiguous().to(dev, torch.float32)
        lw, lb = model.logits.fold()
        self.logit_w = lw[:, :, 0, 0].reshape(lw.shape[0], 1, 1, -1).contiguous().to(dev, torch.bfloat16)
        self.logit_b = lb.to(dev, torch.float32)
        self.head = None
        self._side_streams: List[torch.cuda.Stream] = []
        self._span_tables: Dict[tuple, dict] = {}

    @staticmethod
    def _pack_mnv2_block(blk, dev) -> dict:
        s = blk.spec
        d = dict(
            spec=s, module=blk,
            expand=_pack_dense(blk.expand, dev) if blk.expand is not None else None,
            dw=_pack_dw(blk.dw, dev),
            project=_pack_dense(blk.project, dev))
        row_ok = s.dilation == 1 and s.cin <= 64 and s.cout <= 96 and s.cin % 8 == 0
        shape = (-(-s.cout // 16), -(-s.cin // 32))
        tile_ok = s.cin % 8 == 0 and (
            shape in K.FUSED_TILE_SHAPES if blk.expand is not None
            else shape in K.FUSED_TILE_SHAPES_NOEXP and not s.residual)
        fold = _fold_block(blk)
        if row_ok or tile_ok:
            packed = K.pack_fused_ir(*fold, Cin=s.cin, hid=s.hidden, Cout=s.cout, stride=s.stride,
                                     residual=s.residual, device=dev, dil=s.dilation)
            if row_ok:
                d["fused"] = packed
            if tile_ok:
                d["fused_tile"] = packed
        if s.hidden % 32 == 0 and blk.expand is not None and not row_ok:
            d["dwproj"] = K.pack_project_padded(fold[4], fold[5], s.cout, s.hidden, dev)
        return d

    def _build(self, B: int, Hc: int, Wc: int, buf, bufs):
        mnv2 = self.kind == "mnv2"
        self._cam = (Hc, Wc)
        ops, st = (self._stem_mnv2 if mnv2 else self._stem_resnet)(B, Hc, Wc, buf, bufs)
        first = 1 if mnv2 and self.stem_block0 is not None else 0
        for i in range(first, len(self.blocks)):
            bops, st = (self._mnv2_block if mnv2 else self._resnet_block)(buf, i, self.blocks[i], B, *st)
            ops += bops
        cat = buf("aspp_cat", B, st[1], st[2], self.cat_c)
        branches = self._aspp_branches(B, buf, bufs, cat, *st)
        fork, pool, img_bias = self._aspp_pool(B, buf, bufs, *st)
        ops += fork + branches + pool
        head, logits = self._head(B, buf, cat, img_bias, st[1], st[2])
        return ops + head + self._upsample(B, buf, logits, st[1], st[2])

    def _stem_op(self, B, Hc, Wc, buf, bufs):
        H, W = self.H, self.W
        sw, sb, sk, ss, sact, sc = self.stem
        OH, OW = conv_out_hw(H, W, sk, ss, 1)
        x = buf("stem", B, OH, OW, sc)
        bufs["_in_shape"] = torch.tensor([B, Hc, Wc])
        return (lambda frames, lx, ly: K.stem_conv(
            frames, lx, ly, sw, sb, x, H=H, W=W, OH=OH, OW=OW, Cout=sc, k=sk, stride=ss,
            act=sact)), (x, OH, OW, sc)

    def _stem_resnet(self, B, Hc, Wc, buf, bufs):
        (sw, sb, sk, ss, sact, sc), H, W = self.stem, self.H, self.W
        stem, (x, h, w, c) = self._stem_op(B, Hc, Wc, buf, bufs)
        if (sc, sk) == (64, 7):
            wpk = K.pack_stem_mfma(sw, sk, sc)
            bufs["const_stem_wpk"] = wpk
            stem = Choice("stem", [("fp32", [stem])] + [(f"mfmaw{tile[0]}x{tile[1]}", [
                lambda frames, lx, ly, tile=tile: K.stem_mfma(
                    frames, lx, ly, wpk, sb, x, H=H, W=W, OH=h, OW=w, Cout=sc, k=sk, stride=ss,
                    act=sact, tile=tile, per_wave=True)]) for tile in ((16, 32), (32, 32))])
        PH, PW = conv_out_hw(h, w, 3, 2, 1)
        y = buf("pool0", B, PH, PW, c)
        pool = (lambda *_: K.maxpool3x3s2(x, y, B=B, IH=h, IW=w, C=c, OH=PH, OW=PW))
        return [stem, pool], (y, PH, PW, c)

    def _stem_mnv2(self, B, Hc, Wc, buf, bufs):
        H, W = self.H, self.W
        stem, st = self._stem_op(B, Hc, Wc, buf, bufs)
        if self.stem_block0 is None:
            return [stem], st
        block0, st0 = self._mnv2_block(buf, 0, self.blocks[0], B, *st)
        sbp, out0, SH = self.stem_block0, st0[0], st[1]
        tiles = [(f"stem_block0_{ty}x{tx}", [
            lambda frames, lx, ly, ty=ty, tx=tx: K.stem_block0(
                frames, lx, ly, sbp, out0, H=H, W=W, tile=(ty, tx))])
            for ty, tx in ((8, 16), (4, 16), (8, 8), (16, 16), (8, 32), (12, 16))]
        bands: Dict[str, List[Callable]] = {}
        for nbx in (3, 4, 5):
            Rs = [max(2, -(-B * nbx * SH // target)) for target in (256, 512, 1024)]
            Rs += [max(2, -(-SH // nby)) for nby in range(2, 13)
                   if B * nbx * nby in range(640, 800) or B * nbx * nby in range(1400, 1560)]
            for R in dict.fromkeys(Rs):
                for oneb in (True, False):
                    bands.setdefault(f"stem_band{R}x{nbx}" + ("" if oneb else "b2"), [
                        lambda frames, lx, ly, R=R, nbx=nbx, oneb=oneb: K.stem_band(
                            frames, lx, ly, sbp, out0, H=H, W=W, R=R, nbx=nbx, one_barrier=oneb,
                            row_repeat=self._row_repeat(0, SH, R))])
        return [Choice("stem+block0", list(bands.items())[::-1] + tiles +
                       [("separate", [stem] + block0)])], st0

    def _aspp_branches(self, B, buf, bufs, cat, x, h, w, c):
        A = self.aspp_c
        b0w, b0b = self.aspp_b0
        sep = [pw_choice("aspp.b0", lambda *_: K.conv_gemm(
            x, b0w, b0b, cat, B=B, IH=h, IW=w, Cin=c, OH=h, OW=w, Cout=A, k=1, ldo=self.cat_c,
            co_off=0, act="relu"), x, b0w, b0b, cat, M=B * h * w, Cin=c, Cout=A, ldo=self.cat_c,
            co_off=0, act="relu")]
        for j, ((aw, ab), rate) in enumerate(self.aspp_atrous):
            variants = []
            if c in K.TAP_CIN and A % 8 == 0:
                twp, tbp = K.pack_tap_weights(aw, ab)
                for name, grouped in (("tap", False), ("tapg", True)):
                    perm = K.tap_group_perm(B, h, w, 3, rate, 256, self.device) if grouped else None
                    variants.append((name, [
                        lambda *_, twp=twp, tbp=tbp, rate=rate, j=j, perm=perm:
                        K.tap_conv(x, twp, tbp, cat, B=B, H=h, W=w, Cin=c, Cout=A, k=3, dil=rate,
                                   ldo=self.cat_c, co_off=(j + 1) * A, act="relu", perm=perm)]))
            for name, variant, bm in (("v4", 4, 0), ("v4g", 4, 128), ("v5g", 5, 128),
                                      ("v6g", 6, 256)):
                perm = K.tap_group_perm(B, h, w, 3, rate, bm, self.device) if bm else None
                variants.append((name, [
                    lambda *_, aw=aw, ab=ab, rate=rate, j=j, variant=variant, perm=perm: K.conv_gemm(
                        x, aw, ab, cat, B=B, IH=h, IW=w, Cin=c, OH=h, OW=w, Cout=A, k=3, dil=rate,
                        ldo=self.cat_c, co_off=(j + 1) * A, act="relu", variant=variant,
                        perm=perm)]))
            sep.append(Choice(f"aspp.rate{rate}", variants))
        if len(self.aspp_atrous) <= 3 and c % 8 == 0:
            return [Choice("aspp.branches",
                           self._aspp_grouped(B, buf, bufs, cat, x, h, w, c) + [("separate", sep)])]
        return sep

    def _aspp_grouped(self, B, buf, bufs, cat, x, h, w, c):
        A, dev = self.aspp_c, self.device
        b0w, b0b = self.aspp_b0
        grouped = []
        for gv in (5, 6, 8, 12, 13, 14, 15, 16, 17, 18):
            BM = K.GROUP_TILE[gv][0]
            convs = [dict(x=x, w=b0w, bias=b0b, out=cat, B=B, IH=h, IW=w, Cin=c, OH=h, OW=w,
                          Cout=A, k=1, dil=1, ldo=self.cat_c, co_off=0, act="relu")]
            for j, ((aw, ab), rate) in enumerate(self.aspp_atrous):
                convs.append(dict(x=x, w=aw, bias=ab, out=cat, B=B, IH=h, IW=w, Cin=c, OH=h,
                                  OW=w, Cout=A, k=3, dil=rate, ldo=self.cat_c,
                                  co_off=(j + 1) * A, act="relu",
                                  perm=K.tap_group_perm(B, h, w, 3, rate, BM, dev)))
            order = K.grouped_tile_order(convs, gv, dev)
            bufs[f"aspp_order{gv}"] = order
            grouped.append((f"grouped_v{gv}", [
                lambda *_, convs=convs, order=order, gv=gv: K.conv_gemm_grouped(convs, order, gv)]))
            ks_opts = (2, 4, 6) if B <= 2 else (2, 3) if B <= 8 else ()
            if ks_opts and gv in (5, 17, 18) and A * (len(self.aspp_atrous) + 1) == self.cat_c:
                if "aspp_part" not in bufs:
                    buf("aspp_part", max(ks_opts) * B * h * w * self.cat_c, dtype=torch.float32)
                    bufs["const_aspp_bias_cat"] = torch.cat(
                        [b0b.float()] + [ab.float() for (_, ab), _ in self.aspp_atrous]).to(dev).contiguous()
                ntile = max(-(-(cv["perm"].numel() if cv.get("perm") is not None else B * h * w) // BM)
                            for cv in convs) * -(-A // K.GROUP_TILE[gv][1])
                cnt = buf(f"aspp_cnt{gv}", 4 * ntile, dtype=torch.int32)
                for ks in ks_opts:
                    order_k = K.grouped_tile_order(convs, gv, dev, ks=ks)
                    bufs[f"aspp_order{gv}k{ks}"] = order_k
                    for inl in (False, True):
                        grouped.append((f"grouped_v{gv}k{ks}" + ("c" if inl else ""), [
                            lambda *_, convs=convs, order=order_k, gv=gv, ks=ks, cnt=(cnt if inl else None):
                            K.conv_gemm_grouped(convs, order, gv, ks=ks, part=bufs["aspp_part"],
                                                bias_cat=bufs["const_aspp_bias_cat"], cnt=cnt)]))
        return grouped

    def _aspp_pool(self, B, buf, bufs, x, h, w, c):
        if not self.has_pool:
            return [], [], None
        A, dev = self.aspp_c, self.device
        img_bias = buf("img_bias", B, A, dtype=torch.float32)
        gws = K.gap_workspace(B, c, dev)
        bufs["gap_ws"] = gws
        if not (c <= 2048 and A <= 512 and c % 8 == 0 and A % 4 == 0):
            gap = buf("gap", B, c, dtype=torch.float32)
            pooled = buf("pooled", B, A, dtype=torch.float32)
            return [], [
                lambda *_: K.global_avgpool(x, gap, B=B, HW=h * w, C=c, ws=gws),
                lambda *_: K.matvec(gap, self.pool_w, self.pool_b, pooled, B=B, N=A, K=c, act="relu"),
                lambda *_: K.matvec(pooled, self.proj_pool_w, None, img_bias, B=B, N=A, K=A)], img_bias
        w1t = self.pool_w.t().contiguous()
        w2t = self.proj_pool_w.t().contiguous()
        bufs["pool_w1t"], bufs["pool_w2t"] = w1t, w2t
        pool_op = (lambda *_: K.aspp_pool(
            x, gws, w1t, self.pool_b, w2t, img_bias, B=B, HW=h * w, C=c, N=A))
        if not (os.environ.get("SSA_POOL_FORK", "0") == "1" and torch.cuda.is_available()):
            return [], [pool_op], img_bias
        side = torch.cuda.Stream(dev)
        ev_f, ev_j = torch.cuda.Event(), torch.cuda.Event()
        self._side_streams.append(side)

        def fork_op(*args):
            ev_f.record(torch.cuda.current_stream())
            side.wait_event(ev_f)
            with torch.cuda.stream(side):
                pool_op(*args)
            ev_j.record(side)

        return [fork_op], [lambda *_: torch.cuda.current_stream().wait_event(ev_j)], img_bias

    def _head(self, B, buf, cat, img_bias, h, w):
        A = self.aspp_c
        proj = buf("aspp_proj", B, h, w, A)
        proj_variants = [(f"v{v}", [
            lambda *_, v=v: K.conv_gemm(
                cat, self.proj_w, self.proj_b, proj, B=B, IH=h, IW=w, Cin=self.cat_c, OH=h, OW=w,
                Cout=A, k=1, act="relu", img_bias=img_bias, variant=v)]) for v in (4, 3, 5, 6)]
        logits = buf("logits", B, h, w, self.ldk)
        split = [Choice("aspp.proj", proj_variants), pw_choice("logits", lambda *_: K.conv_gemm(
            proj, self.logit_w, self.logit_b, logits, B=B, IH=h, IW=w, Cin=A, OH=h, OW=w,
            Cout=self.num_classes, k=1, ldo=self.ldk, act=None), proj, self.logit_w,
            self.logit_b, logits, M=B * h * w, Cin=A, Cout=self.num_classes, ldo=self.ldk, act=None,
            N_out=self.ldk)]
        if not (A == 256 and self.cat_c == 1024 and self.num_classes <= 32 and self.ldk <= 32):
            return split, logits
        if self.head is None:
            self.head = K.pack_aspp_head(self.proj_w, self.proj_b, self.logit_w, self.logit_b, self.device)
        Mh = B * h * w
        g0 = K.aspp_head_groups(Mh)
        head = [(f"head_g{g}" + ("w" if nw == 16 else ""), [lambda *_, g=g, nw=nw: K.aspp_head(
            cat.view(Mh, self.cat_c), self.head, logits.view(Mh, self.ldk), M=Mh, HW=h * w,
            ldo=self.ldk, img_bias=img_bias, G=g, waves=nw)]) for g in K.ASPP_HEAD_G
            if g == g0 or (g < g0 and -(-Mh // (16 * g)) <= 1024) for nw in (8, 16)]
        return [Choice("aspp.head", head + [("split", split)])], logits

    def _upsample(self, B, buf, logits, h, w):
        H, W = self.H, self.W
        labels = buf("labels", B, H, W, dtype=torch.uint8)
        return [Choice("upsample", [(name, [lambda *_, v=K.UPSAMPLE_VARIANTS[name]: K.upsample_argmax(
            logits, self._labels_out if self._labels_out is not None else labels, B=B, h=h, w=w,
            K=self.num_classes, ldk=self.ldk, H=H, W=W, variant=v)])
            for name in ("rows", "lane", "union", "cand")])]

    def _mnv2_block(self, buf, i, blk, B, x, h, w, c):
        s = blk["spec"]
        hid = s.hidden
        unfused: List[Callable] = []
        e = x
        if blk["expand"] is not None:
            ew, eb = blk["expand"]
            e = buf(f"b{i}_exp", B, h, w, hid)
            unfused.append(pw_choice(f"block{i}.expand", lambda *_: K.conv_gemm(
                x, ew, eb, e, B=B, IH=h, IW=w, Cin=c, OH=h, OW=w, Cout=hid, k=1, act="relu6"),
                x, ew, eb, e, M=B * h * w, Cin=c, Cout=hid, act="relu6"))
        OH, OW = conv_out_hw(h, w, 3, s.stride, s.dilation)
        dw_w, dw_b = blk["dw"]
        d = buf(f"b{i}_dw", B, OH, OW, hid)
        unfused.append(lambda *_: K.depthwise3x3(
            e, dw_w, dw_b, d, B=B, IH=h, IW=w, C=hid, OH=OH, OW=OW, stride=s.stride,
            dil=s.dilation, act="relu6"))
        pw_, pb_ = blk["project"]
        out = buf(f"b{i}_out", B, OH, OW, s.cout)
        res = x if s.residual else None
        unfused.append(lambda *_: K.conv_gemm(
            d, pw_, pb_, out, B=B, IH=OH, IW=OW, Cin=hid, OH=OH, OW=OW, Cout=s.cout, k=1,
            act=None, res=res))
        g = SimpleNamespace(i=i, blk=blk, s=s, B=B, x=x, h=h, w=w, c=c, hid=hid, e=e, out=out,
                            res=res, OH=OH, OW=OW, buf=buf, expand_op=unfused[0])
        dwp, dwproj, tile = self._dwp_variants(g), self._dwproj_variants(g), self._tile_variants(g)
        stream, band, slices = self._stream_variants(g), self._band_variants(g), self._slice_variants(g)
        variants = slices + band + stream + tile + [("unfused", unfused)] + dwp + dwproj
        return [Choice(f"block{i}", variants)], (out, OH, OW, s.cout)

    def _dwp_variants(self, g):
        s, blk, B, h, w, c, hid, OH, OW = g.s, g.blk, g.B, g.h, g.w, g.c, g.hid, g.OH, g.OW
        if not (blk["expand"] is not None and hid % 32 == 0 and s.cout in K.DWP_COUT
                and K.pw_supported(c, hid)):
            return []
        ew, eb = blk["expand"]
        (pw_, pb_), (dw_w, dw_b) = blk["project"], blk["dw"]
        e16 = g.buf(f"b{g.i}_exp16", B, h, w, hid, dtype=torch.float16)
        ewpk = K.pack_pw_weights(ew, eb)
        wpk_dp = K.pack_dw_proj(pw_[:, 0, 0, :], dw_w, dw_b)
        M = B * h * w
        cfgs = [("w", 4, 0, 2, False)]
        if s.stride == 1:
            cfgs += [("r", 4, ty, 2, False) for ty in (2, 3, 4)]
            cfgs += [("r", 4, ty, st, True) for ty in (2, 3, 4, 6) for st in (2, 3, 4)
                     if _dwp_rows_fit(ty, st, s.dilation, OW, s.cout)]
        out = []
        for mt, nch in ((2, 3),):
            for kind, nw, ty, st, xcd in cfgs:
                tag = f"dwp{kind}{nw if not ty else ty}" + (f"s{st}x" if xcd else "")
                out.append((f"{tag}.pw{mt}x{nch}", [
                    lambda *_, mt=mt, nch=nch: K.pw_conv(
                        g.x, ewpk, e16, M=M, K=c, N=hid, act="relu6", mt=mt, nch=nch),
                    lambda *_, nw=nw, ty=ty, st=st, xcd=xcd:
                    K.dw_proj_fused(e16, wpk_dp, pb_, g.out, B=B, IH=h, IW=w, hid=hid,
                                    Cout=s.cout, OH=OH, OW=OW, stride=s.stride,
                                    dil=s.dilation, res=g.res, waves=nw, rows=ty, stages=st,
                                    xcd=xcd)]))
        return out

    def _dwproj_variants(self, g):
        if "dwproj" not in g.blk:
            return []
        s, (dpw, dpb), (dw_w, dw_b) = g.s, g.blk["dwproj"], g.blk["dw"]
        return [("dwproj", [g.expand_op, lambda *_: K.dw_project(
            g.e, dw_w, dw_b, dpw, dpb, g.out, B=g.B, IH=g.h, IW=g.w, hid=g.hid, Cout=s.cout,
            OH=g.OH, OW=g.OW, stride=s.stride, dil=s.dilation, res=g.res)])]

    def _tile_variants(self, g):
        s, blk = g.s, g.blk
        geom = dict(B=g.B, IH=g.h, IW=g.w, OH=g.OH, OW=g.OW)
        out = []
        if "fused_tile" in blk:
            fp = blk["fused_tile"]
            for tile in _tile_candidates(g.OH, g.OW, fp["CinP"], s.stride, s.dilation,
                                         fp["we"] is not None):
                out.append((f"tile{tile[0]}x{tile[1]}", [
                    lambda *_, fp=fp, tile=tile: K.fused_ir(g.x, fp, g.out, tile=tile, **geom)]))
        if "fused" in blk:
            out.append(("fused", [lambda *_, fp=blk["fused"]: K.fused_ir(g.x, fp, g.out, **geom)]))
        return out[::-1]

    def _stream_variants(self, g):
        s, blk, B, h, w = g.s, g.blk, g.B, g.h, g.w
        if not (blk["expand"] is not None and s.stride == 1 and (s.cin, s.cout) in FS.STREAM_SHAPES):
            return []
        narrow = s.cout <= 96 and s.dilation == 1
        out = []

        def stream(name, tab, v, **kw):
            sp = self._packed(blk, "span")
            out.append((name, [lambda *_: FS.fused_ir_stream(
                g.x, sp, tab, g.out, B=B, residual=s.residual, variant=v, **kw)]))

        for S in self._span_counts(B, h, w):
            if FS.stream_supported(s.cin, s.cout, 1, h, w, S, s.dilation, lattice=True):
                ltab = self._span_table(h, w, S, s.dilation, lattice=True)
                for v in ((0, 1, 2, 4) if s.cout <= 160 else (1,)):
                    stream(f"stream{S}" + {0: "", 1: "g", 2: "w", 4: "r3"}[v] + "L", ltab, v)
                self._split_hidden(g, S, stream, ltab, [(0 if s.cout <= 160 else 1, "L")])
            if FS.stream_supported(s.cin, s.cout, 1, h, w, S, s.dilation):
                tab = self._span_table(h, w, S, s.dilation)
                vs = ((0, 1, 2) if narrow else (0, 1)) + \
                    ((4,) if s.cout <= 160 else ()) + ((6,) if narrow else ())
                for v in vs:
                    stream(f"stream{S}" + {0: "", 1: "g", 2: "w", 4: "r3", 6: "wr3"}[v], tab, v)
                self._split_hidden(g, S, stream, tab, [(0, ""), (2, "w")] if narrow else [(0, "")])
        return out[::-1]

    @staticmethod
    def _split_hidden(g, S, stream, tab, kernels) -> None:
        s, B, i = g.s, g.B, g.i
        nc = -(-g.hid // 32)
        hs_opts = [hs for hs in (2, 3, 4, 6) if hs <= nc and B * S * hs <= 512] if B <= 16 else []
        if not hs_opts:
            return
        if not hasattr(g, "part"):
            g.part = g.buf(f"b{i}_part", max(hs_opts) * B * g.h * g.w * s.cout, dtype=torch.float32)
        cnt = g.buf(f"b{i}_cnt{S}", B * S, dtype=torch.int32)
# ... 117 lines not shown
```

### semantic_segmentation_server_amd/ops/hip_ops.py

```python
from __future__ import annotations

from typing import List, Optional

import os

import torch

from .native import hip as _hip_mod

ACT = {None: 0, "none": 0, "relu": 1, "relu6": 2}


_DEBUG_SYNC = os.environ.get("SSA_DEBUG_SYNC", "0") == "1"


def _stream() -> int:
    return torch._C._cuda_getCurrentRawStream(torch._C._cuda_getDevice())


def _dbg(name: str, **shapes) -> None:
    if not _DEBUG_SYNC or torch.cuda.is_current_stream_capturing():
        return
    try:
        torch.cuda.synchronize()
    except Exception as e:
        raise RuntimeError(f"kernel {name} failed with {shapes}: {e}") from e


def _ptr(t: Optional[torch.Tensor]) -> int:
    return 0 if t is None else t.data_ptr()


def _chk(t: torch.Tensor, dtype, name: str, numel: Optional[int] = None) -> None:
    if t.dtype != dtype:
        raise TypeError(f"{name}: expected {dtype}, got {t.dtype}")
    if not t.is_cuda:
        raise ValueError(f"{name}: must be a CUDA tensor")
    if not t.is_contiguous():
        raise ValueError(f"{name}: must be contiguous")
    if numel is not None and t.numel() < numel:
        raise ValueError(f"{name}: has {t.numel()} elements, kernel needs {numel}")


def conv_out_hw(IH: int, IW: int, k: int, stride: int, dil: int):
    pad = dil * (k // 2)
    OH = (IH + 2 * pad - dil * (k - 1) - 1) // stride + 1
    OW = (IW + 2 * pad - dil * (k - 1) - 1) // stride + 1
    return OH, OW


def conv_gemm(x: torch.Tensor, w: torch.Tensor, bias: torch.Tensor, out: torch.Tensor, *,
              B: int, IH: int, IW: int, Cin: int, OH: int, OW: int, Cout: int, k: int = 1,
              stride: int = 1, dil: int = 1, ldo: Optional[int] = None, co_off: int = 0,
              act=None, res: Optional[torch.Tensor] = None, ldr: Optional[int] = None,
              img_bias: Optional[torch.Tensor] = None, variant: int = 0,
              perm: Optional[torch.Tensor] = None) -> torch.Tensor:
    ldo = Cout if ldo is None else ldo
    ldr = Cout if ldr is None else ldr
    if Cin % 8:
        raise ValueError("conv_gemm: Cin must be a multiple of 8")
    if co_off + Cout > ldo:
        raise ValueError("conv_gemm: co_off + Cout > ldo")
    _chk(x, torch.bfloat16, "x", B * IH * IW * Cin)
    _chk(w, torch.bfloat16, "w", Cout * k * k * Cin)
    _chk(bias, torch.float32, "bias", Cout)
    _chk(out, torch.bfloat16, "out", B * OH * OW * ldo)
    if res is not None:
        _chk(res, torch.bfloat16, "res", B * OH * OW * ldr)
    if img_bias is not None:
        _chk(img_bias, torch.float32, "img_bias", B * Cout)
    Mp = 0
    if perm is not None:
        _chk(perm, torch.int32, "perm")
        Mp = perm.numel()
        if variant not in (3, 4, 5, 6, 8, 9, 10):
            raise ValueError("conv_gemm: perm needs an LDS-DMA variant (3-6, 8-10)")
        if not getattr(perm, "_ssa_checked", False):
            pc = perm.cpu()
            if pc.min().item() < -1 or pc.max().item() >= B * OH * OW:
                raise ValueError("conv_gemm: perm entry out of range")
            perm._ssa_checked = True
    _hip_mod().conv_gemm(_ptr(x), _ptr(w), _ptr(bias), _ptr(img_bias), _ptr(res), _ptr(out), B, IH,
                         IW, Cin, OH, OW, Cout, k, k, stride, dil, ldo, co_off, ldr, ACT[act],
                         _stream(), variant, _ptr(perm), Mp)
    _dbg('conv_gemm')
    return out


def tap_group_perm(B: int, H: int, W: int, k: int, dil: int, BM: int, device=None) -> torch.Tensor:
    r = dil * (k // 2)

    def cls(n):
        i = torch.arange(n)
        return (i - r < 0).long() * 2 + (i + r > n - 1).long()

    key = (cls(H)[:, None] * 4 + cls(W)[None, :]).reshape(-1)
    order = []
    for c in torch.unique(key).tolist():
        px = torch.nonzero(key == c).flatten()
        idx = (torch.arange(B)[:, None] * (H * W) + px[None, :]).reshape(-1)
        pad = (-idx.numel()) % BM
        order.append(idx)
        if pad:
            order.append(torch.full((pad,), -1, dtype=torch.long))
    return torch.cat(order).to(torch.int32).to(device).contiguous()


GROUP_TILE = {5: (128, 256), 6: (256, 256), 8: (128, 256), 10: (128, 128), 11: (128, 128),
              12: (256, 256), 13: (128, 256), 14: (256, 256), 15: (256, 256), 16: (256, 256),
              17: (128, 256), 18: (256, 128)}


def _tile_taps(B: int, H: int, W: int, k: int, dil: int, BM: int,
               perm: Optional[torch.Tensor]) -> torch.Tensor:
    r = dil * (k // 2)
    ys, xs = torch.arange(H), torch.arange(W)
    bits = torch.zeros(H, W, dtype=torch.long)
    for t in range(k * k):
        dy, dx = (t // k) * dil - r, (t % k) * dil - r
        oky = ((ys + dy >= 0) & (ys + dy < H))[:, None]
        okx = ((xs + dx >= 0) & (xs + dx < W))[None, :]
        bits |= (oky & okx).long() << t
    rows = bits.reshape(-1).repeat(B)
    if perm is not None:
        pc = perm.cpu().long()
        rows = torch.where(pc >= 0, rows[pc.clamp(min=0)], torch.zeros_like(pc))
    pad = (-rows.numel()) % BM
    rows = torch.cat([rows, torch.zeros(pad, dtype=torch.long)]).reshape(-1, BM)
    tile = torch.zeros(rows.shape[0], dtype=torch.long)
    for j in range(BM):
        tile |= rows[:, j]
    return sum(((tile >> t) & 1) for t in range(k * k))


def grouped_tile_order(convs: List[dict], variant: int, device=None, xcds: int = 1, ks: int = 1) -> torch.Tensor:
    BM, BN = GROUP_TILE[variant]
    ent, cost, part = [], [], []
    for g, c in enumerate(convs):
        tn = -(-c["Cout"] // BN)
        taps = _tile_taps(c["B"], c["OH"], c["OW"], c["k"], c["dil"], BM, c.get("perm"))
        kch = -(-c["Cin"] // 64)
        ntm = taps.numel()
        for tm in range(ntm):
            for n in range(tn):
                stages = int(taps[tm]) * kch
                for sl in range(ks):
                    ent.append((g << 24) | (sl << 20) | (tm * tn + n))
                    cost.append((sl + 1) * stages // ks - sl * stages // ks)
                    part.append(min(xcds - 1, tm * xcds // max(1, ntm)))
    if xcds <= 1:
        idx = sorted(range(len(ent)), key=lambda i: (-cost[i], i))
        return torch.tensor([ent[i] for i in idx], dtype=torch.int32).to(device).contiguous()
    lists = [sorted((i for i in range(len(ent)) if part[i] == x), key=lambda i: (-cost[i], i))
             for x in range(xcds)]
    out, j = [], 0
    while any(j < len(lst) for lst in lists):
        for x in range(xcds):
            if j < len(lists[x]):
                out.append(ent[lists[x][j]])
            else:
                donor = max(range(xcds), key=lambda y: len(lists[y]) - j)
                if len(lists[donor]) > j + 1:
                    out.append(ent[lists[donor].pop()])
        j += 1
    assert sorted(out) == sorted(ent)
    return torch.tensor(out, dtype=torch.int32).to(device).contiguous()


def grouped_tile_order_branch(convs: List[dict], variant: int, device=None, xcds: int = 8) -> torch.Tensor:
    BM, BN = GROUP_TILE[variant]
    tiles = []
    for g, c in enumerate(convs):
        tn = -(-c["Cout"] // BN)
        taps = _tile_taps(c["B"], c["OH"], c["OW"], c["k"], c["dil"], BM, c.get("perm"))
        kch = -(-c["Cin"] // 64)
        for tm in range(taps.numel()):
            for n in range(tn):
                tiles.append((int(taps[tm]) * kch, (g << 24) | (tm * tn + n), g))
    G = len(convs)
    return _branch_affine(tiles, [g for g in range(G) if convs[g]["k"] > 1] or list(range(G)), xcds, device)


def _branch_affine(tiles, heavy, xcds, device):
    gcost = {g: sum(t[0] for t in tiles if t[2] == g) for g in heavy}
    tot = max(1, sum(gcost.values()))
    share = {g: xcds * gcost[g] / tot for g in heavy}
    cnt = {g: max(1, int(share[g])) for g in heavy}
    while sum(cnt.values()) > xcds:
        i = max((g for g in heavy if cnt[g] > 1), key=lambda g: cnt[g] - share[g])
        cnt[i] -= 1
    while sum(cnt.values()) < xcds:
        i = max(heavy, key=lambda g: share[g] - cnt[g])
        cnt[i] += 1
    xs, x0 = {}, 0
    for g in heavy:
        xs[g] = list(range(x0, x0 + cnt[g]))
        x0 += cnt[g]
    T = len(tiles)
    cap = [T // xcds + (1 if x < T % xcds else 0) for x in range(xcds)]
    lists = [[] for _ in range(xcds)]
    load = [0] * xcds
    order = sorted(tiles, key=lambda t: (-t[0], t[1]))
    for cost, ent, g in order:
        if g not in xs:
            continue
        cands = [y for y in xs[g] if len(lists[y]) < cap[y]] or [y for y in range(xcds) if len(lists[y]) < cap[y]]
        x = min(cands, key=lambda y: load[y])
        lists[x].append((cost, ent))
        load[x] += cost
    for cost, ent, g in order:
        if g in xs:
            continue
        x = min((y for y in range(xcds) if len(lists[y]) < cap[y]), key=lambda y: load[y])
        lists[x].append((cost, ent))
        load[x] += cost
    for lst in lists:
        lst.sort(key=lambda t: (-t[0], t[1]))
    out = []
    for j in range(max(cap)):
        for x in range(xcds):
            if j < len(lists[x]):
                out.append(lists[x][j][1])
    assert sorted(out) == sorted(t[1] for t in tiles)
    return torch.tensor(out, dtype=torch.int32).to(device).contiguous()


def conv_gemm_grouped(convs: List[dict], order: torch.Tensor, variant: int = 5, ks: int = 1,
                      part: Optional[torch.Tensor] = None, bias_cat: Optional[torch.Tensor] = None,
                      cnt: Optional[torch.Tensor] = None) -> None:
    if not 1 <= len(convs) <= 4:
        raise ValueError("conv_gemm_grouped: 1..4 convs")
    if variant not in GROUP_TILE:
        raise ValueError(f"conv_gemm_grouped: variant must be one of {sorted(GROUP_TILE)}")
    BM, BN = GROUP_TILE[variant]
    tiles = []
    groups = []
    for c in convs:
        B, IH, IW, Cin, OH, OW, Cout, k = (c[n] for n in ("B", "IH", "IW", "Cin", "OH", "OW", "Cout", "k"))
        dil, ldo, co_off = c.get("dil", 1), c.get("ldo", Cout), c.get("co_off", 0)
        if Cin % 8 or k * k > 16 or Cout != convs[0]["Cout"] or (OH, OW) != (IH, IW):
            raise ValueError("conv_gemm_grouped: stride-1 'same' convs, Cin % 8 == 0, <= 16 taps, one Cout")
        if co_off + Cout > ldo:
            raise ValueError("conv_gemm_grouped: co_off + Cout > ldo")
        _chk(c["x"], torch.bfloat16, "x", B * IH * IW * Cin)
        _chk(c["w"], torch.bfloat16, "w", Cout * k * k * Cin)
        _chk(c["bias"], torch.float32, "bias", Cout)
        _chk(c["out"], torch.bfloat16, "out", B * OH * OW * ldo)
        perm = c.get("perm")
        Mp = 0
        if perm is not None:
            _chk(perm, torch.int32, "perm")
            Mp = perm.numel()
            if Mp % BM:
                raise ValueError("conv_gemm_grouped: perm rows must be a multiple of the tile height")
            if not getattr(perm, "_ssa_checked", False):
                pc = perm.cpu()
                if pc.min().item() < -1 or pc.max().item() >= B * OH * OW:
                    raise ValueError("conv_gemm_grouped: perm entry out of range")
                perm._ssa_checked = True
        M = Mp or B * OH * OW
        tiles.append(-(-M // BM) * -(-Cout // BN))
        groups.append((_ptr(c["x"]), _ptr(c["w"]), _ptr(c["bias"]), 0, 0, _ptr(c["out"]), B, IH, IW,
                       Cin, OH, OW, Cout, k, k, 1, dil, ldo, co_off, Cout, ACT[c.get("act")],
                       _ptr(perm), Mp))
    _chk(order, torch.int32, "order")
    if not getattr(order, "_ssa_checked", False):
        oc = order.cpu().long()
        g, t, sl = oc >> 24, oc & 0xFFFFF, (oc >> 20) & 15
        lim = torch.tensor(tiles)[g.clamp(0, len(tiles) - 1)]
        if (g < 0).any() or (g >= len(convs)).any() or (t >= lim).any() or (sl >= ks).any():
            raise ValueError("conv_gemm_grouped: order entry out of range")
        if oc.numel() != sum(tiles) * ks:
            raise ValueError("conv_gemm_grouped: the order table must list every tile's K slices once")
        order._ssa_checked = True
    if ks > 1:
        c0 = convs[0]
        ldo, Mo = c0.get("ldo", c0["Cout"]), c0["B"] * c0["OH"] * c0["OW"]
        if part is None or bias_cat is None:
            raise ValueError("conv_gemm_grouped: split-K needs part and bias_cat")
        if len({c.get("act") for c in convs}) != 1 or c0.get("act") not in (None, "relu"):
            raise ValueError("conv_gemm_grouped: split-K needs one activation (none / relu)")
        if sorted(c.get("co_off", 0) for c in convs) != list(range(0, ldo, c0["Cout"])):
            raise ValueError("conv_gemm_grouped: split-K convs must tile the output channels")
        if any(c["out"].data_ptr() != c0["out"].data_ptr() or c.get("ldo", c["Cout"]) != ldo for c in convs):
            raise ValueError("conv_gemm_grouped: split-K convs must share one output")
        _chk(part, torch.float32, "part", ks * Mo * ldo)
        _chk(bias_cat, torch.float32, "bias_cat", ldo)
        if cnt is not None:
            _chk(cnt, torch.int32, "cnt", 4 * max(tiles))
    _hip_mod().conv_gemm_grouped(groups, _ptr(order), order.numel(), variant, _stream(), int(ks),
                                 _ptr(part) if ks > 1 else 0, _ptr(cnt) if (ks > 1 and cnt is not None) else 0,
                                 max(tiles))
    _dbg('conv_gemm_grouped')
    if ks > 1 and cnt is None:
        _hip_mod().stream_combine(_ptr(part), _ptr(bias_cat), 0, _ptr(c0["out"]), int(ks), Mo, ldo, _stream(),
                                  1 if c0.get("act") == "relu" else 0)
        _dbg('stream_combine')


def bias_act(x, bias, out, *, M: int, N: int, HW: int = 1, img_bias=None, act=None):
    _chk(x, torch.bfloat16, "x", M * N)
    _chk(out, torch.bfloat16, "out", M * N)
    _chk(bias, torch.float32, "bias", N)
    if img_bias is not None:
        _chk(img_bias, torch.float32, "img_bias", (M // HW) * N)
        if M % HW:
            raise ValueError("bias_act: M must be a multiple of HW")
    if N % 8:
        raise ValueError("bias_act: N must be a multiple of 8")
    _hip_mod().bias_act(_ptr(x), _ptr(bias), _ptr(img_bias), _ptr(out), M, N, HW, ACT[act], _stream())
    _dbg('bias_act')
    return out


def pw_supported(K: int, N: int) -> bool:
    ks = (K + 31) // 32
    return K % 8 == 0 and N % 8 == 0 and (ks <= 5 or ks in (8, 10))


def pack_pw_weights(w: torch.Tensor, bias: torch.Tensor, N_out: Optional[int] = None) -> torch.Tensor:
    w = w.reshape(w.shape[0], -1).float()
    N, Kd = w.shape
    Np = max(N, N_out or N)
    NC, KS = -(-Np // 64), -(-Kd // 32)
    full = torch.zeros(NC * 64, KS * 32, dtype=torch.float32, device=w.device)
    full[:N, :Kd] = w
    wt = full.reshape(NC, 4, 16, KS, 4, 8).permute(0, 1, 3, 4, 2, 5).reshape(NC, -1)
    bt = torch.zeros(NC, 256, dtype=torch.float32, device=w.device)
    bflat = torch.zeros(NC * 64, dtype=torch.float32, device=w.device)
    bflat[:N] = bias.float().to(w.device)
    bt[:, :64] = bflat.reshape(NC, 64)
    return torch.cat([wt.to(torch.bfloat16), bt.view(torch.bfloat16)], dim=1).contiguous()


def pw_conv(x, wpk, out, *, M, K, N, ldo=None, co_off=0, act=None, res=None, ldr=None,
            img_bias=None, HW=1, mt=2, nch=1) -> torch.Tensor:
    ldo = N if ldo is None else ldo
    ldr = N if ldr is None else ldr
    if not pw_supported(K, N) or ldo % 8 or co_off % 8 or (res is not None and ldr % 8):
        raise ValueError(f"pw_conv: unsupported K={K} N={N} ldo={ldo} co_off={co_off}")
    if co_off + N > ldo or mt not in (2, 4) or nch < 1:
        raise ValueError("pw_conv: bad co_off / mt / nch")
    NC, KS = -(-N // 64), -(-K // 32)
    _chk(x, torch.bfloat16, "x", M * K)
    _chk(wpk, torch.bfloat16, "wpk", NC * (4 * KS + 1) * 512)
    out_f16 = out.dtype == torch.float16
    _chk(out, torch.float16 if out_f16 else torch.bfloat16, "out", M * ldo)
    if res is not None:
        _chk(res, torch.bfloat16, "res", M * ldr)
    if img_bias is not None:
        _chk(img_bias, torch.float32, "img_bias", (M // HW) * N)
        if M % HW:
            raise ValueError("pw_conv: M must be a multiple of HW with img_bias")
    _hip_mod().pw_conv(_ptr(x), _ptr(wpk), _ptr(img_bias), _ptr(res), _ptr(out), M, K, N, HW, ldo,
                       co_off, ldr, ACT[act], mt, nch, _stream(), int(out_f16))
    _dbg('pw_conv')
    return out


TAP_GROUP = 128
TAP_CIN = (64, 128, 160, 256, 320)


def pack_tap_weights(w: torch.Tensor, bias: torch.Tensor):
    Cout, kh, kw, Cin = w.shape
    T, G, KS = kh * kw, -(-Cout // TAP_GROUP), -(-Cin // 32)
    full = torch.zeros(T, G * TAP_GROUP, KS * 32, dtype=torch.float32, device=w.device)
    full[:, :Cout, :Cin] = w.float().reshape(Cout, T, Cin).permute(1, 0, 2)
    packed = full.reshape(T, G, 8, 16, KS, 4, 8).permute(0, 1, 2, 4, 5, 3, 6).contiguous()
    b = torch.zeros(G * TAP_GROUP, dtype=torch.float32, device=w.device)
    b[:Cout] = bias.float()
    return packed.to(torch.bfloat16).reshape(-1), b


def tap_conv(x, wpk, bias_p, out, *, B, H, W, Cin, Cout, k=3, dil=1, ldo=None, co_off=0, act=None,
             perm: Optional[torch.Tensor] = None) -> torch.Tensor:
    ldo = Cout if ldo is None else ldo
    if Cin not in TAP_CIN or Cout % 8 or ldo % 8 or co_off % 8 or co_off + Cout > ldo:
        raise ValueError(f"tap_conv: unsupported Cin={Cin} Cout={Cout} ldo={ldo} co_off={co_off}")
    G = -(-Cout // TAP_GROUP)
    _chk(x, torch.bfloat16, "x", B * H * W * Cin)
    _chk(wpk, torch.bfloat16, "wpk", k * k * G * TAP_GROUP * (-(-Cin // 32)) * 32)
    _chk(bias_p, torch.float32, "bias", G * TAP_GROUP)
    _chk(out, torch.bfloat16, "out", B * H * W * ldo)
    Mp = 0
    if perm is not None:
        _chk(perm, torch.int32, "perm")
        Mp = perm.numel()
        if not getattr(perm, "_ssa_checked", False):
            pc = perm.cpu()
            if pc.min().item() < -1 or pc.max().item() >= B * H * W:
                raise ValueError("tap_conv: perm entry out of range")
            perm._ssa_checked = True
    _hip_mod().tap_conv(_ptr(x), _ptr(wpk), _ptr(bias_p), _ptr(out), _ptr(perm), Mp, B, H, W, Cin,
                        Cout, k, k, dil, ldo, co_off, ACT[act], _stream())
    _dbg('tap_conv')
    return out


def fused_ir(x, packed: dict, out, *, B, IH, IW, OH, OW, tile=None, trace=None):
    P = packed
    TY, TX = tile if tile is not None else (0, 0)
    if tile is None and P.get("dil", 1) != 1:
        raise ValueError("fused_ir: dilated blocks need the tile kernel")
    _chk(x, torch.bfloat16, "x", B * IH * IW * P["Cin"])
    _chk(out, torch.bfloat16, "out", B * OH * OW * P["Cout"])
    if P["we"] is not None:
        _chk(P["we"], torch.bfloat16, "we", P["hidP"] * P["CinP"])
    _chk(P["wd"], torch.float32, "wd", 9 * P["hidP"])
    _chk(P["wp"], torch.bfloat16, "wp", P["CoutP"] * P["hidP"])
    exp_oh = (IH - 1) // P["stride"] + 1
    if (OH, OW) != (exp_oh, (IW - 1) // P["stride"] + 1):
        raise ValueError("fused_ir: output size mismatch")
    _hip_mod().fused_ir(_ptr(x), _ptr(P["we"]), _ptr(P["be"]), _ptr(P["wd"]), _ptr(P["bd"]),
                        _ptr(P["wp"]), _ptr(P["bp"]), _ptr(out), B, IH, IW, P["Cin"], P["CinP"],
                        P["hidP"], P["Cout"], OH, OW, P["stride"], int(P["residual"]), _stream(),
                        P.get("dil", 1), TY, TX, _ptr(P["wd_h"]), _ptr(P["bd_h"]), _ptr(P["wp_h"]),
                        _ptr(trace))
    _dbg('fused_ir')
    return out


def dw_project(hid_in, wd, bd, wp, bp, out, *, B, IH, IW, hid, Cout, OH, OW, stride=1, dil=1,
               res=None):
    CoutP = (Cout + 15) // 16 * 16
    if hid % 32:
        raise ValueError("dw_project: hid must be a multiple of 32")
    _chk(hid_in, torch.bfloat16, "hid_in", B * IH * IW * hid)
    _chk(wd, torch.float32, "wd", 9 * hid)
    _chk(bd, torch.float32, "bd", hid)
    _chk(wp, torch.bfloat16, "wp", CoutP * hid)
    _chk(bp, torch.float32, "bp", CoutP)
    _chk(out, torch.bfloat16, "out", B * OH * OW * Cout)
    if res is not None:
        _chk(res, torch.bfloat16, "res", B * OH * OW * Cout)
    _hip_mod().dw_project(_ptr(hid_in), _ptr(wd), _ptr(bd), _ptr(wp), _ptr(bp), _ptr(res), _ptr(out),
                          B, IH, IW, hid, Cout, OH, OW, stride, dil, _stream())
    _dbg('dw_project')
    return out


DWP_COUT = (64, 96, 160, 320)


def pack_dw_proj(wp: torch.Tensor, wd9: torch.Tensor, bd: torch.Tensor) -> torch.Tensor:
# ... 605 lines not shown
```

Before: 39070 frames/s.

## Fold ASPP image-pool work items into the grouped conv GEMM launch

Adds pool work items (global average pool, then two small matvecs) as extra entries at the head of the grouped ASPP conv tile order. One kernel launch now does both the ASPP branch convs and the image-pooling branch, with one block per image using the conv kernel's LDS. This removes a separate pool kernel launch and lets the pool run alongside the conv tiles. The cost is extra validation, LDS fit constraints and only a few allowed variants, and a single block per image doing the whole reduction could become a long straggler.

Measured after the change: 39660 frames/s (median of 6 runs). +1.5%, better.

```diff
diff --git a/csrc/hip/aspp_pool.h b/csrc/hip/aspp_pool.h
--- /dev/null
+++ b/csrc/hip/aspp_pool.h
@@ -0,0 +1,171 @@
+#pragma once
+#include "common.h"
+
+namespace ssa {
+
+constexpr int kGapSlices = 32;
+constexpr int kPoolMaxC = 2048, kPoolMaxN = 512;
+constexpr int kPoolVT = 1024;
+
+__device__ __forceinline__ void gap_slice_range(int HW, int sl, int& p0, int& p1) {
+  p0 = (int)((long long)HW * sl / kGapSlices);
+  p1 = (int)((long long)HW * (sl + 1) / kGapSlices);
+}
+
+template <int NCH, int U>
+__device__ __forceinline__ void gap_chains(const bf16* __restrict__ base, int C, int p, int p1,
+                                           float (&acc)[NCH][8]) {
+  for (; p + 4 * (U - 1) + NCH - 1 < p1; p += 4 * U) {
+    bf16x8 v[U][NCH];
+#pragma unroll
+    for (int u = 0; u < U; ++u)
+#pragma unroll
+      for (int c = 0; c < NCH; ++c) v[u][c] = ld8(base + (long long)(p + 4 * u + c) * C);
+#pragma unroll
+    for (int u = 0; u < U; ++u)
+#pragma unroll
+      for (int c = 0; c < NCH; ++c)
+#pragma unroll
+        for (int q = 0; q < 8; ++q) acc[c][q] += (float)v[u][c][q];
+  }
+  for (; p < p1; p += 4) {
+    bf16x8 v[NCH];
+#pragma unroll
+    for (int c = 0; c < NCH; ++c) v[c] = ld8(base + (long long)(p + c < p1 ? p + c : p) * C);
+#pragma unroll
+    for (int c = 0; c < NCH; ++c)
+      if (p + c < p1) {
+#pragma unroll
+        for (int q = 0; q < 8; ++q) acc[c][q] += (float)v[c][q];
+      }
+  }
+}
+
+__device__ __forceinline__ float4 pool_slice(const float* __restrict__ wt, const float* s_x, int k0,
+                                             int k1, int N, int q) {
+  float4 a0 = make_float4(0.f, 0.f, 0.f, 0.f), a1 = a0;
+  int k = k0;
+  for (; k + 2 <= k1; k += 2) {
+    const float4 w0 = *reinterpret_cast<const float4*>(wt + (size_t)k * N + 4 * q);
+    const float4 w1 = *reinterpret_cast<const float4*>(wt + (size_t)(k + 1) * N + 4 * q);
+    const float x0 = s_x[k], x1 = s_x[k + 1];
+    a0.x += w0.x * x0; a0.y += w0.y * x0; a0.z += w0.z * x0; a0.w += w0.w * x0;
+    a1.x += w1.x * x1; a1.y += w1.y * x1; a1.z += w1.z * x1; a1.w += w1.w * x1;
+  }
+  if (k < k1) {
+    const float4 w0 = *reinterpret_cast<const float4*>(wt + (size_t)k * N + 4 * q);
+    const float x0 = s_x[k];
+    a0.x += w0.x * x0; a0.y += w0.y * x0; a0.z += w0.z * x0; a0.w += w0.w * x0;
+  }
+  return make_float4(a0.x + a1.x, a0.y + a1.y, a0.z + a1.z, a0.w + a1.w);
+}
+
+template <int VT>
+__device__ __forceinline__ void aspp_pool_mlp(const float* __restrict__ part,
+                                              const float* __restrict__ w1t,
+                                              const float* __restrict__ b1,
+                                              const float* __restrict__ w2t, float* __restrict__ out,
+                                              int HW, int C, int N, float* s_gap, float* s_pool,
+                                              float4* s_red, int tid, int nthr, float* dimg, float4* dv) {
+  const float inv = 1.f / (float)HW;
+  for (int k = tid; k < C; k += nthr) {
+    float s = 0.f;
+#pragma unroll
+    for (int q = 0; q < kGapSlices; ++q) s += part[(size_t)q * C + k];
+    s_gap[k] = s * inv;
+  }
+  const int nq = N >> 2;
+  const int nks = VT / nq;
+  __syncthreads();
+  if (dimg)
+    for (int k = tid; k < C; k += nthr) dimg[k] = s_gap[k];
+  {
+    const int per = (C + nks - 1) / nks;
+    for (int vt = tid; vt < VT; vt += nthr) {
+      const int q = vt % nq, ks = vt / nq;
+      const int k0 = min(C, ks * per), k1 = min(C, k0 + per);
+      if (ks < nks) {
+        const float4 r = pool_slice(w1t, s_gap, k0, k1, N, q);
+        s_red[ks * nq + q] = r;
+        if (dv) dv[vt] = r;
+      }
+    }
+  }
+  __syncthreads();
+  if (tid < nq) {
+    float4 s = s_red[tid];
+    if (dv) dv[VT + tid] = s;
+    for (int j = 1; j < nks; ++j) {
+      const float4 v = s_red[j * nq + tid];
+      if (dv) dv[VT + j * nq + tid] = v;
+      s.x += v.x; s.y += v.y; s.z += v.z; s.w += v.w;
+    }
+    s_pool[4 * tid + 0] = fmaxf(s.x + b1[4 * tid + 0], 0.f);
+    s_pool[4 * tid + 1] = fmaxf(s.y + b1[4 * tid + 1], 0.f);
+    s_pool[4 * tid + 2] = fmaxf(s.z + b1[4 * tid + 2], 0.f);
+    s_pool[4 * tid + 3] = fmaxf(s.w + b1[4 * tid + 3], 0.f);
+  }
+  __syncthreads();
+  if (dimg)
+    for (int k = tid; k < N; k += nthr) dimg[C + k] = s_pool[k];
+  {
+    const int per = (N + nks - 1) / nks;
+    for (int vt = tid; vt < VT; vt += nthr) {
+      const int q = vt % nq, ks = vt / nq;
+      const int k0 = min(N, ks * per), k1 = min(N, k0 + per);
+      if (ks < nks) {
+        const float4 r = pool_slice(w2t, s_pool, k0, k1, N, q);
+        s_red[ks * nq + q] = r;
+        if (dv) dv[2 * VT + vt] = r;
+      }
+    }
+  }
+  __syncthreads();
+  if (tid < nq) {
+    float4 s = s_red[tid];
+    if (dv) dv[3 * VT + tid] = s;
+    for (int j = 1; j < nks; ++j) {
+      const float4 v = s_red[j * nq + tid];
+      if (dv) dv[3 * VT + j * nq + tid] = v;
+      s.x += v.x; s.y += v.y; s.z += v.z; s.w += v.w;
+    }
+    *reinterpret_cast<float4*>(out + 4 * tid) = s;
+  }
+}
+
+__host__ __device__ constexpr size_t pool_item_lds(int C, int N) {
+  return ((size_t)(kGapSlices + 1) * C + N) * 4 + (size_t)kPoolVT * 16;
+}
+
+template <int NTHR>
+__device__ __forceinline__ void aspp_pool_item(const bf16* __restrict__ in ,
+                                               const float* __restrict__ w1t,
+                                               const float* __restrict__ b1,
+                                               const float* __restrict__ w2t, float* __restrict__ out,
+                                               int HW, int C, int N, char* smem) {
+  float* s_part = reinterpret_cast<float*>(smem);
+  float* s_gap = s_part + (size_t)kGapSlices * C;
+  float* s_pool = s_gap + C;
+  float4* s_red = reinterpret_cast<float4*>(s_pool + N);
+  const int tid = threadIdx.x;
+  const int CG = C >> 3;
+  for (int it = tid; it < kGapSlices * CG; it += NTHR) {
+    const int sl = it / CG, cg = it - sl * CG;
+    int p0, p1;
+    gap_slice_range(HW, sl, p0, p1);
+    float acc[4][8];
+#pragma unroll
+    for (int c = 0; c < 4; ++c)
+#pragma unroll
+      for (int q = 0; q < 8; ++q) acc[c][q] = 0.f;
+    gap_chains<4, 2>(in + cg * 8, C, p0, p1, acc);
+    float* dst = s_part + (size_t)sl * C + cg * 8;
+#pragma unroll
+    for (int q = 0; q < 8; ++q) dst[q] = acc[0][q] + acc[1][q] + acc[2][q] + acc[3][q];
+  }
+  __syncthreads();
+  aspp_pool_mlp<kPoolVT>(s_part, w1t, b1, w2t, out, HW, C, N, s_gap, s_pool, s_red, tid, NTHR,
+                         nullptr, nullptr);
+}
+
+}
diff --git a/csrc/hip/bindings.cpp b/csrc/hip/bindings.cpp
--- a/csrc/hip/bindings.cpp
+++ b/csrc/hip/bindings.cpp
@@ -38,7 +38,7 @@
 
   m.def("conv_gemm_grouped",
         [](py::list groups, uintptr_t order, int nblocks, int variant, uintptr_t stream, int ks, uintptr_t part,
-           uintptr_t cnt, int cnt_stride) {
+           uintptr_t cnt, int cnt_stride, py::object pool) {
           std::vector<ConvParams> ps;
           for (auto item : groups) {
             auto t = item.cast<py::tuple>();
@@ -54,12 +54,23 @@
             p.perm = P<const int>(U(21)); p.Mp = I(22);
             ps.push_back(p);
           }
+          GroupPoolParams gp;
+          if (!pool.is_none()) {
+            auto t = pool.cast<py::tuple>();
+            if (t.size() != 9) throw std::invalid_argument("conv_gemm_grouped: 9-tuple for pool");
+            auto U = [&](int i) { return t[i].cast<uintptr_t>(); };
+            gp.in = P<const bf16>(U(0)); gp.w1t = P<const float>(U(1)); gp.b1 = P<const float>(U(2));
+            gp.w2t = P<const float>(U(3)); gp.img_bias = P<float>(U(4));
+            gp.B = t[5].cast<int>(); gp.HW = t[6].cast<int>(); gp.C = t[7].cast<int>();
+            gp.N = t[8].cast<int>();
+          }
           conv_gemm_grouped(ps.data(), (int)ps.size(), P<const int>(order), nblocks, variant,
-                            S(stream), ks, P<float>(part), P<int>(cnt), cnt_stride);
+                            S(stream), ks, P<float>(part), P<int>(cnt), cnt_stride,
+                            pool.is_none() ? nullptr : &gp);
         },
         py::arg("groups"), py::arg("order"), py::arg("nblocks"), py::arg("variant"),
         py::arg("stream"), py::arg("ks") = 1, py::arg("part") = 0, py::arg("cnt") = 0,
-        py::arg("cnt_stride") = 0);
+        py::arg("cnt_stride") = 0, py::arg("pool") = py::none());
 
   m.def("bias_act", [](uintptr_t in, uintptr_t bias, uintptr_t img_bias, uintptr_t out, long long M,
                        int N, int HW, int act, uintptr_t stream) {
diff --git a/csrc/hip/conv_gemm.hip b/csrc/hip/conv_gemm.hip
--- a/csrc/hip/conv_gemm.hip
+++ b/csrc/hip/conv_gemm.hip
@@ -1,3 +1,4 @@
+#include "aspp_pool.h"
 #include "common.h"
 #include "kernels.h"
 
@@ -14,6 +15,11 @@
 };
 
 constexpr int kMaxConvGroup = 4;
+constexpr int kPoolGroup = kMaxConvGroup;
+struct PoolArgs {
+  const bf16* in; const float* w1t; const float* b1; const float* w2t; float* img_bias;
+  int B, HW, C, N;
+};
 struct ConvGroupArgs {
   ConvArgs g[kMaxConvGroup];
   const int* order;
@@ -22,6 +28,12 @@
   int* cnt;
   int cnt_stride;
 };
+struct ConvGroupPoolArgs {
+  ConvGroupArgs ga;
+  PoolArgs pool;
+};
+template <int MT, int NT, int ST, int WM, int WN, int BK>
+constexpr bool kGroupPoolOk = WM * WN >= 8 && BK == 64 && NT == 4;
 
 template <int MT, int NT>
 __global__ __launch_bounds__(256) void conv_gemm_kernel(ConvArgs a) {
@@ -705,10 +717,54 @@
 }
 
 template <int MT, int NT, int ST, int WM = 2, int WN = 2, int BK = 64>
-static void launch_conv_glds_group(const ConvGroupArgs& ga, int nblocks, hipStream_t s) {
+__global__ __launch_bounds__(64 * WM * WN) void conv_glds_group_pool_kernel(ConvGroupPoolArgs gp) {
+  extern __shared__ __attribute__((aligned(16))) char smem[];
+  const int e = __builtin_amdgcn_readfirstlane(gp.ga.order[blockIdx.x]);
+  const int t = e & 0xfffff, ksl = (e >> 20) & 15;
+  switch (e >> 24) {
+    case 0: glds_tile<MT, NT, ST, WM, WN, BK>(gp.ga.g[0], t, smem, gp.ga.ks, ksl, gp.ga.part, gp.ga.cnt); break;
+    case 1: glds_tile<MT, NT, ST, WM, WN, BK>(gp.ga.g[1], t, smem, gp.ga.ks, ksl, gp.ga.part,
+                                              gp.ga.cnt ? gp.ga.cnt + gp.ga.cnt_stride : nullptr); break;
+    case 2: glds_tile<MT, NT, ST, WM, WN, BK>(gp.ga.g[2], t, smem, gp.ga.ks, ksl, gp.ga.part,
+                                              gp.ga.cnt ? gp.ga.cnt + 2 * gp.ga.cnt_stride : nullptr); break;
+    case 3: glds_tile<MT, NT, ST, WM, WN, BK>(gp.ga.g[3], t, smem, gp.ga.ks, ksl, gp.ga.part,
+                                              gp.ga.cnt ? gp.ga.cnt + 3 * gp.ga.cnt_stride : nullptr); break;
+    case kPoolGroup:
+      if (t < gp.pool.B)
+        aspp_pool_item<64 * WM * WN>(gp.pool.in + (size_t)t * gp.pool.HW * gp.pool.C, gp.pool.w1t,
+                                     gp.pool.b1, gp.pool.w2t, gp.pool.img_bias + (size_t)t * gp.pool.N,
+                                     gp.pool.HW, gp.pool.C, gp.pool.N, smem);
+      break;
+    default: break;
+  }
+}
+
+template <int MT, int NT, int ST, int WM = 2, int WN = 2, int BK = 64>
+static void launch_conv_glds_group(const ConvGroupArgs& ga, int nblocks, hipStream_t s,
+                                   const PoolArgs* pool = nullptr) {
   constexpr int BM = 16 * MT * WM, BN = 16 * NT * WN;
   const size_t lds = (size_t)ST * (BM + BN) * BK * 2 + 16;
   static_assert((size_t)ST * (BM + BN) * BK * 2 + 16 <= 160 * 1024, "LDS ring too large");
+  if (pool) {
+    if constexpr (kGroupPoolOk<MT, NT, ST, WM, WN, BK>) {
+      if (pool_item_lds(pool->C, pool->N) > lds)
+        throw std::invalid_argument("conv_gemm_grouped: the pool work item does not fit this variant's LDS");
+      static bool pool_attr_set = false;
+      if (!pool_attr_set) {
+        check(hipFuncSetAttribute(
+                  reinterpret_cast<const void*>(&conv_glds_group_pool_kernel<MT, NT, ST, WM, WN, BK>),
+                  hipFuncAttributeMaxDynamicSharedMemorySize, 160 * 1024),
+              "conv_glds_group_pool attr");
+        pool_attr_set = true;
+      }
+      hipLaunchKernelGGL((conv_glds_group_pool_kernel<MT, NT, ST, WM, WN, BK>), dim3(nblocks),
+                         dim3(64 * WM * WN), lds, s, ConvGroupPoolArgs{ga, *pool});
+      check_launch("conv_glds_group_pool");
+      return;
+    } else {
+      throw std::invalid_argument("conv_gemm_grouped: this variant carries no pool work items");
+    }
+  }
   static bool attr_set = false;
   if (!attr_set) {
     check(hipFuncSetAttribute(reinterpret_cast<const void*>(&conv_glds_group_kernel<MT, NT, ST, WM, WN, BK>),
@@ -859,7 +915,8 @@
 }
 
 void conv_gemm_grouped(const ConvParams* ps, int n, const int* order, int nblocks, int variant,
-                       hipStream_t s, int ks, float* part, int* cnt, int cnt_stride) {
+                       hipStream_t s, int ks, float* part, int* cnt, int cnt_stride,
+                       const GroupPoolParams* pool) {
   if (n < 1 || n > kMaxConvGroup) throw std::invalid_argument("conv_gemm_grouped: 1..4 convs");
   if (!order || nblocks < 1) throw std::invalid_argument("conv_gemm_grouped: empty tile order");
   if (ks < 1 || ks > 16 || (ks > 1 && part == nullptr))
@@ -883,19 +940,29 @@
     ga.g[i] = to_args(p);
   }
   ga.order = order;
+  PoolArgs pa{};
+  if (pool) {
+    const GroupPoolParams& q = *pool;
+    if (!q.in || !q.w1t || !q.b1 || !q.w2t || !q.img_bias || q.B < 1 || q.HW < 1)
+      throw std::invalid_argument("conv_gemm_grouped: pool operands missing");
+    if (q.C > kPoolMaxC || q.N > kPoolMaxN || q.C % 8 || q.N % 4 || q.C < 8 || q.N < 4)
+      throw std::invalid_argument("conv_gemm_grouped: pool needs C <= 2048, C % 8, N <= 512, N % 4");
+    pa = PoolArgs{q.in, q.w1t, q.b1, q.w2t, q.img_bias, q.B, q.HW, q.C, q.N};
+  }
+  const PoolArgs* pp = pool ? &pa : nullptr;
   switch (variant) {
-    case 5: launch_conv_glds_group<4, 4, 2, 2, 4>(ga, nblocks, s); break;
-    case 6: launch_conv_glds_group<8, 4, 2, 2, 4>(ga, nblocks, s); break;
-    case 8: launch_conv_glds_group<4, 4, 3, 2, 4>(ga, nblocks, s); break;
-    case 10: launch_conv_glds_group<4, 4, 4, 2, 2>(ga, nblocks, s); break;
-    case 11: launch_conv_glds_group<4, 4, 2, 2, 2>(ga, nblocks, s); break;
-    case 12: launch_conv_glds_group<8, 4, 4, 2, 4, 32>(ga, nblocks, s); break;
-    case 13: launch_conv_glds_group<4, 4, 4, 2, 4, 32>(ga, nblocks, s); break;
-    case 14: launch_conv_glds_group<8, 4, 3, 2, 4, 32>(ga, nblocks, s); break;
-    case 15: launch_conv_glds_group<4, 4, 2, 4, 4>(ga, nblocks, s); break;
-    case 16: launch_conv_glds_group<4, 4, 4, 4, 4, 32>(ga, nblocks, s); break;
-    case 17: launch_conv_glds_group<2, 4, 2, 4, 4>(ga, nblocks, s); break;
-    case 18: launch_conv_glds_group<4, 2, 2, 4, 4>(ga, nblocks, s); break;
+    case 5: launch_conv_glds_group<4, 4, 2, 2, 4>(ga, nblocks, s, pp); break;
+    case 6: launch_conv_glds_group<8, 4, 2, 2, 4>(ga, nblocks, s, pp); break;
+    case 8: launch_conv_glds_group<4, 4, 3, 2, 4>(ga, nblocks, s, pp); break;
+    case 10: launch_conv_glds_group<4, 4, 4, 2, 2>(ga, nblocks, s, pp); break;
+    case 11: launch_conv_glds_group<4, 4, 2, 2, 2>(ga, nblocks, s, pp); break;
+    case 12: launch_conv_glds_group<8, 4, 4, 2, 4, 32>(ga, nblocks, s, pp); break;
+    case 13: launch_conv_glds_group<4, 4, 4, 2, 4, 32>(ga, nblocks, s, pp); break;
+    case 14: launch_conv_glds_group<8, 4, 3, 2, 4, 32>(ga, nblocks, s, pp); break;
+    case 15: launch_conv_glds_group<4, 4, 2, 4, 4>(ga, nblocks, s, pp); break;
+    case 16: launch_conv_glds_group<4, 4, 4, 4, 4, 32>(ga, nblocks, s, pp); break;
+    case 17: launch_conv_glds_group<2, 4, 2, 4, 4>(ga, nblocks, s, pp); break;
+    case 18: launch_conv_glds_group<4, 2, 2, 4, 4>(ga, nblocks, s, pp); break;
     default: throw std::invalid_argument("conv_gemm_grouped: variant must be 5, 6, 8, 10-18");
   }
 }
diff --git a/csrc/hip/kernels.h b/csrc/hip/kernels.h
--- a/csrc/hip/kernels.h
+++ b/csrc/hip/kernels.h
@@ -21,9 +21,15 @@
   int Mp = 0;
 };
 void conv_gemm(const ConvParams& p, hipStream_t s);
+struct GroupPoolParams {
+  const bf16* in = nullptr;
+  const float* w1t = nullptr; const float* b1 = nullptr; const float* w2t = nullptr;
+  float* img_bias = nullptr;
+  int B = 0, HW = 0, C = 0, N = 0;
+};
 void conv_gemm_grouped(const ConvParams* ps, int n, const int* order, int nblocks, int variant,
                        hipStream_t s, int ks = 1, float* part = nullptr, int* cnt = nullptr,
-                       int cnt_stride = 0);
+                       int cnt_stride = 0, const GroupPoolParams* pool = nullptr);
 
 struct PwConvParams {
   const bf16* in = nullptr;
diff --git a/csrc/hip/model_ops.hip b/csrc/hip/model_ops.hip
--- a/csrc/hip/model_ops.hip
+++ b/csrc/hip/model_ops.hip
@@ -1,3 +1,4 @@
+#include "aspp_pool.h"
 #include "common.h"
 #include "kernels.h"
 
@@ -454,8 +455,6 @@
   check_launch("maxpool3x3s2");
 }
 
-constexpr int kGapSlices = 32;
-
 __global__ __launch_bounds__(256) void gap_partial_kernel(const bf16* __restrict__ in,
                                                           float* __restrict__ part, int HW, int C) {
   const int b = blockIdx.x, sl = blockIdx.y;
@@ -463,28 +462,13 @@
   const int lane = threadIdx.x & 63, wid = threadIdx.x >> 6;
   const int cg = blockIdx.z * 64 + lane;
   __shared__ float red[4][64][8];
-  float acc[8] = {0, 0, 0, 0, 0, 0, 0, 0};
-  const int p0 = (int)((long long)HW * sl / kGapSlices), p1 = (int)((long long)HW * (sl + 1) / kGapSlices);
-  if (cg < CG) {
-    const bf16* base = in + (long long)b * HW * C + cg * 8;
-    int p = p0 + wid;
-    for (; p + 12 < p1; p += 16) {
-      bf16x8 v[4];
-#pragma unroll
-      for (int u = 0; u < 4; ++u) v[u] = ld8(base + (long long)(p + 4 * u) * C);
-#pragma unroll
-      for (int u = 0; u < 4; ++u)
-#pragma unroll
-        for (int q = 0; q < 8; ++q) acc[q] += (float)v[u][q];
-    }
-    for (; p < p1; p += 4) {
-      const bf16x8 v = ld8(base + (long long)p * C);
-#pragma unroll
-      for (int q = 0; q < 8; ++q) acc[q] += (float)v[q];
-    }
-  }
-#pragma unroll
-  for (int q = 0; q < 8; ++q) red[wid][lane][q] = acc[q];
+  float acc[1][8] = {{0, 0, 0, 0, 0, 0, 0, 0}};
+  int p0, p1;
+  gap_slice_range(HW, sl, p0, p1);
+  if (cg < CG)
+    gap_chains<1, 4>(in + (long long)b * HW * C + cg * 8, C, p0 + wid, p1, acc);
+#pragma unroll
+  for (int q = 0; q < 8; ++q) red[wid][lane][q] = acc[0][q];
   __syncthreads();
   if (wid == 0 && cg < CG) {
 #pragma unroll
@@ -621,27 +605,6 @@
   check_launch("matvec");
 }
 
-constexpr int kPoolMaxC = 2048, kPoolMaxN = 512;
-
-__device__ __forceinline__ float4 pool_slice(const float* __restrict__ wt, const float* s_x, int k0,
-                                             int k1, int N, int q) {
-  float4 a0 = make_float4(0.f, 0.f, 0.f, 0.f), a1 = a0;
-  int k = k0;
-  for (; k + 2 <= k1; k += 2) {
-    const float4 w0 = *reinterpret_cast<const float4*>(wt + (size_t)k * N + 4 * q);
-    const float4 w1 = *reinterpret_cast<const float4*>(wt + (size_t)(k + 1) * N + 4 * q);
-    const float x0 = s_x[k], x1 = s_x[k + 1];
-    a0.x += w0.x * x0; a0.y += w0.y * x0; a0.z += w0.z * x0; a0.w += w0.w * x0;
-    a1.x += w1.x * x1; a1.y += w1.y * x1; a1.z += w1.z * x1; a1.w += w1.w * x1;
-  }
-  if (k < k1) {
-    const float4 w0 = *reinterpret_cast<const float4*>(wt + (size_t)k * N + 4 * q);
-    const float x0 = s_x[k];
-    a0.x += w0.x * x0; a0.y += w0.y * x0; a0.z += w0.z * x0; a0.w += w0.w * x0;
-  }
-  return make_float4(a0.x + a1.x, a0.y + a1.y, a0.z + a1.z, a0.w + a1.w);
-}
-
 template <int kPoolThreads>
 __global__ __launch_bounds__(kPoolThreads) void aspp_pool_kernel(const float* __restrict__ part,
                                                                  const float* __restrict__ w1t,
@@ -653,70 +616,12 @@
   if (mode & 1) __builtin_amdgcn_fence(__ATOMIC_ACQUIRE, "agent");
   __shared__ float s_pool[kPoolMaxN];
   __shared__ float4 s_red[kPoolThreads];
-  const int b = blockIdx.x, tid = threadIdx.x;
-  const float inv = 1.f / (float)HW;
-  const float* pb = part + (size_t)b * kGapSlices * C;
-  for (int k = tid; k < C; k += kPoolThreads) {
-    float s = 0.f;
-#pragma unroll
-    for (int q = 0; q < kGapSlices; ++q) s += pb[(size_t)q * C + k];
-    s_gap[k] = s * inv;
-  }
-  const int nq = N >> 2;
-  const int nks = kPoolThreads / nq;
-  const int q = tid % nq, ks = tid / nq;
-  __syncthreads();
+  const int b = blockIdx.x;
   const size_t dstride = (size_t)C + N + 4 * 4 * kPoolThreads;
   float* dimg = dbg ? dbg + (size_t)b * dstride : nullptr;
   float4* dv = dbg ? reinterpret_cast<float4*>(dimg + C + N) : nullptr;
-  if (dbg)
-    for (int k = tid; k < C; k += kPoolThreads) dimg[k] = s_gap[k];
-  {
-    const int per = (C + nks - 1) / nks;
-    const int k0 = min(C, ks * per), k1 = min(C, k0 + per);
-    if (ks < nks) {
-      const float4 r = pool_slice(w1t, s_gap, k0, k1, N, q);
-      s_red[ks * nq + q] = r;
-      if (dbg) dv[tid] = r;
-    }
-  }
-  __syncthreads();
-  if (tid < nq) {
-    float4 s = s_red[tid];
-    if (dbg) dv[kPoolThreads + tid] = s;
-    for (int j = 1; j < nks; ++j) {
-      const float4 v = s_red[j * nq + tid];
-      if (dbg) dv[kPoolThreads + j * nq + tid] = v;
-      s.x += v.x; s.y += v.y; s.z += v.z; s.w += v.w;
-    }
-    s_pool[4 * tid + 0] = fmaxf(s.x + b1[4 * tid + 0], 0.f);
-    s_pool[4 * tid + 1] = fmaxf(s.y + b1[4 * tid + 1], 0.f);
-    s_pool[4 * tid + 2] = fmaxf(s.z + b1[4 * tid + 2], 0.f);
-    s_pool[4 * tid + 3] = fmaxf(s.w + b1[4 * tid + 3], 0.f);
-  }
-  __syncthreads();
-  if (dbg)
-    for (int k = tid; k < N; k += kPoolThreads) dimg[C + k] = s_pool[k];
-  {
-    const int per = (N + nks - 1) / nks;
-    const int k0 = min(N, ks * per), k1 = min(N, k0 + per);
-    if (ks < nks) {
-      const float4 r = pool_slice(w2t, s_pool, k0, k1, N, q);
-      s_red[ks * nq + q] = r;
-      if (dbg) dv[2 * kPoolThreads + tid] = r;
-    }
-  }
-  __syncthreads();
-  if (tid < nq) {
-    float4 s = s_red[tid];
-    if (dbg) dv[3 * kPoolThreads + tid] = s;
-    for (int j = 1; j < nks; ++j) {
-      const float4 v = s_red[j * nq + tid];
-      if (dbg) dv[3 * kPoolThreads + j * nq + tid] = v;
-      s.x += v.x; s.y += v.y; s.z += v.z; s.w += v.w;
-    }
-    *reinterpret_cast<float4*>(img_bias + (size_t)b * N + 4 * tid) = s;
-  }
+  aspp_pool_mlp<kPoolThreads>(part + (size_t)b * kGapSlices * C, w1t, b1, w2t, img_bias + (size_t)b * N,
+                              HW, C, N, s_gap, s_pool, s_red, threadIdx.x, kPoolThreads, dimg, dv);
 }
 
 void aspp_pool(const bf16* in, float* ws, const float* w1t, const float* b1, const float* w2t,
diff --git a/semantic_segmentation_server_amd/models/hip_model.py b/semantic_segmentation_server_amd/models/hip_model.py
--- a/semantic_segmentation_server_amd/models/hip_model.py
+++ b/semantic_segmentation_server_amd/models/hip_model.py
@@ -174,9 +174,8 @@
             bops, st = (self._mnv2_block if mnv2 else self._resnet_block)(buf, i, self.blocks[i], B, *st)
             ops += bops
         cat = buf("aspp_cat", B, st[1], st[2], self.cat_c)
-        branches = self._aspp_branches(B, buf, bufs, cat, *st)
-        fork, pool, img_bias = self._aspp_pool(B, buf, bufs, *st)
-        ops += fork + branches + pool
+        fork, pool, img_bias, item = self._aspp_pool(B, buf, bufs, *st)
+        ops += fork + self._aspp_branches(B, buf, bufs, cat, *st, pool=pool, item=item)
         head, logits = self._head(B, buf, cat, img_bias, st[1], st[2])
         return ops + head + self._upsample(B, buf, logits, st[1], st[2])
 
@@ -230,7 +229,8 @@
         return [Choice("stem+block0", list(bands.items())[::-1] + tiles +
                        [("separate", [stem] + block0)])], st0
 
-    def _aspp_branches(self, B, buf, bufs, cat, x, h, w, c):
+    def _aspp_branches(self, B, buf, bufs, cat, x, h, w, c, pool=(), item=None):
+        pool = list(pool)
         A = self.aspp_c
         b0w, b0b = self.aspp_b0
         sep = [pw_choice("aspp.b0", lambda *_: K.conv_gemm(
@@ -257,14 +257,25 @@
                         perm=perm)]))
             sep.append(Choice(f"aspp.rate{rate}", variants))
         if len(self.aspp_atrous) <= 3 and c % 8 == 0:
-            return [Choice("aspp.branches",
-                           self._aspp_grouped(B, buf, bufs, cat, x, h, w, c) + [("separate", sep)])]
-        return sep
-
-    def _aspp_grouped(self, B, buf, bufs, cat, x, h, w, c):
+            grouped, fused = self._aspp_grouped(B, buf, bufs, cat, x, h, w, c, item)
+            if not fused:
+                return [Choice("aspp.branches", grouped + [("separate", sep)])] + pool
+            return [Choice("aspp.branches", [(n, v + pool) for n, v in grouped] +
+                           [("separate", sep + pool)] + fused)]
+        return sep + pool
+
+    def _aspp_grouped(self, B, buf, bufs, cat, x, h, w, c, item=None):
         A, dev = self.aspp_c, self.device
         b0w, b0b = self.aspp_b0
-        grouped = []
+        grouped, fused = [], []
+
+        def add(name, convs, order, gv, **kw):
+            grouped.append((name, [lambda *_: K.conv_gemm_grouped(convs, order, gv, **kw)]))
+            if item is not None and gv in K.GROUP_POOL_VARIANTS and K.pool_item_fits(gv, item["C"], item["N"]):
+                order_p = K.with_pool_items(order, B)
+                bufs[f"aspp_order{name[len('grouped_v'):]}p"] = order_p
+                fused.append((name + "+pool", [
+                    lambda *_: K.conv_gemm_grouped(convs, order_p, gv, pool=item, **kw)]))
         for gv in (5, 6, 8, 12, 13, 14, 15, 16, 17, 18):
             BM = K.GROUP_TILE[gv][0]
             convs = [dict(x=x, w=b0w, bias=b0b, out=cat, B=B, IH=h, IW=w, Cin=c, OH=h, OW=w,
@@ -276,8 +287,7 @@
                                   perm=K.tap_group_perm(B, h, w, 3, rate, BM, dev)))
             order = K.grouped_tile_order(convs, gv, dev)
             bufs[f"aspp_order{gv}"] = order
-            grouped.append((f"grouped_v{gv}", [
-                lambda *_, convs=convs, order=order, gv=gv: K.conv_gemm_grouped(convs, order, gv)]))
+            add(f"grouped_v{gv}", convs, order, gv)
             ks_opts = (2, 4, 6) if B <= 2 else (2, 3) if B <= 8 else ()
             if ks_opts and gv in (5, 17, 18) and A * (len(self.aspp_atrous) + 1) == self.cat_c:
                 if "aspp_part" not in bufs:
@@ -291,15 +301,14 @@
                     order_k = K.grouped_tile_order(convs, gv, dev, ks=ks)
                     bufs[f"aspp_order{gv}k{ks}"] = order_k
                     for inl in (False, True):
-                        grouped.append((f"grouped_v{gv}k{ks}" + ("c" if inl else ""), [
-                            lambda *_, convs=convs, order=order_k, gv=gv, ks=ks, cnt=(cnt if inl else None):
-                            K.conv_gemm_grouped(convs, order, gv, ks=ks, part=bufs["aspp_part"],
-                                                bias_cat=bufs["const_aspp_bias_cat"], cnt=cnt)]))
-        return grouped
+                        add(f"grouped_v{gv}k{ks}" + ("c" if inl else ""), convs, order_k, gv, ks=ks,
+                            part=bufs["aspp_part"], bias_cat=bufs["const_aspp_bias_cat"],
+                            cnt=cnt if inl else None)
+        return grouped, fused
 
     def _aspp_pool(self, B, buf, bufs, x, h, w, c):
         if not self.has_pool:
-            return [], [], None
+            return [], [], None, None
         A, dev = self.aspp_c, self.device
         img_bias = buf("img_bias", B, A, dtype=torch.float32)
         gws = K.gap_workspace(B, c, dev)
@@ -310,14 +319,15 @@
             return [], [
                 lambda *_: K.global_avgpool(x, gap, B=B, HW=h * w, C=c, ws=gws),
                 lambda *_: K.matvec(gap, self.pool_w, self.pool_b, pooled, B=B, N=A, K=c, act="relu"),
-                lambda *_: K.matvec(pooled, self.proj_pool_w, None, img_bias, B=B, N=A, K=A)], img_bias
+                lambda *_: K.matvec(pooled, self.proj_pool_w, None, img_bias, B=B, N=A, K=A)], img_bias, None
         w1t = self.pool_w.t().contiguous()
         w2t = self.proj_pool_w.t().contiguous()
         bufs["pool_w1t"], bufs["pool_w2t"] = w1t, w2t
         pool_op = (lambda *_: K.aspp_pool(
             x, gws, w1t, self.pool_b, w2t, img_bias, B=B, HW=h * w, C=c, N=A))
         if not (os.environ.get("SSA_POOL_FORK", "0") == "1" and torch.cuda.is_available()):
-            return [], [pool_op], img_bias
+            item = dict(x=x, w1t=w1t, b1=self.pool_b, w2t=w2t, img_bias=img_bias, B=B, HW=h * w, C=c, N=A)
+            return [], [pool_op], img_bias, item if os.environ.get("SSA_POOL_FUSED", "1") != "0" else None
         side = torch.cuda.Stream(dev)
         ev_f, ev_j = torch.cuda.Event(), torch.cuda.Event()
         self._side_streams.append(side)
@@ -329,7 +339,7 @@
                 pool_op(*args)
             ev_j.record(side)
 
-        return [fork_op], [lambda *_: torch.cuda.current_stream().wait_event(ev_j)], img_bias
+        return [fork_op], [lambda *_: torch.cuda.current_stream().wait_event(ev_j)], img_bias, None
 
     def _head(self, B, buf, cat, img_bias, h, w):
         A = self.aspp_c
diff --git a/semantic_segmentation_server_amd/ops/hip_ops.py b/semantic_segmentation_server_amd/ops/hip_ops.py
--- a/semantic_segmentation_server_amd/ops/hip_ops.py
+++ b/semantic_segmentation_server_amd/ops/hip_ops.py
@@ -109,6 +109,10 @@
 GROUP_TILE = {5: (128, 256), 6: (256, 256), 8: (128, 256), 10: (128, 128), 11: (128, 128),
               12: (256, 256), 13: (128, 256), 14: (256, 256), 15: (256, 256), 16: (256, 256),
               17: (128, 256), 18: (256, 128)}
+POOL_GROUP = 4
+GROUP_POOL_VARIANTS = (5, 6, 8, 15, 17)
+GROUP_LDS = {5: 98320, 6: 131088, 8: 147472, 10: 131088, 11: 65552, 12: 131088, 13: 98320,
+             14: 98320, 15: 131088, 16: 131088, 17: 98320, 18: 98320}
 
 
 def _tile_taps(B: int, H: int, W: int, k: int, dil: int, BM: int,
@@ -133,7 +137,8 @@
     return sum(((tile >> t) & 1) for t in range(k * k))
 
 
-def grouped_tile_order(convs: List[dict], variant: int, device=None, xcds: int = 1, ks: int = 1) -> torch.Tensor:
+def grouped_tile_order(convs: List[dict], variant: int, device=None, xcds: int = 1, ks: int = 1,
+                       pool: int = 0) -> torch.Tensor:
     BM, BN = GROUP_TILE[variant]
     ent, cost, part = [], [], []
     for g, c in enumerate(convs):
@@ -150,7 +155,7 @@
                     part.append(min(xcds - 1, tm * xcds // max(1, ntm)))
     if xcds <= 1:
         idx = sorted(range(len(ent)), key=lambda i: (-cost[i], i))
-        return torch.tensor([ent[i] for i in idx], dtype=torch.int32).to(device).contiguous()
+        return with_pool_items(torch.tensor([ent[i] for i in idx], dtype=torch.int32), pool).to(device).contiguous()
     lists = [sorted((i for i in range(len(ent)) if part[i] == x), key=lambda i: (-cost[i], i))
              for x in range(xcds)]
     out, j = [], 0
@@ -164,7 +169,19 @@
                     out.append(ent[lists[donor].pop()])
         j += 1
     assert sorted(out) == sorted(ent)
-    return torch.tensor(out, dtype=torch.int32).to(device).contiguous()
+    return with_pool_items(torch.tensor(out, dtype=torch.int32), pool).to(device).contiguous()
+
+
+def pool_item_fits(variant: int, C: int, N: int) -> bool:
+    return (33 * C + N) * 4 + 16384 <= GROUP_LDS[variant]
+
+
+def with_pool_items(order: torch.Tensor, images: int) -> torch.Tensor:
+    if images <= 0:
+        return order
+    head = torch.tensor([(POOL_GROUP << 24) | b for b in range(images)], dtype=torch.int32,
+                        device=order.device)
+    return torch.cat([head, order]).contiguous()
 
 
 def grouped_tile_order_branch(convs: List[dict], variant: int, device=None, xcds: int = 8) -> torch.Tensor:
@@ -227,7 +244,7 @@
 
 def conv_gemm_grouped(convs: List[dict], order: torch.Tensor, variant: int = 5, ks: int = 1,
                       part: Optional[torch.Tensor] = None, bias_cat: Optional[torch.Tensor] = None,
-                      cnt: Optional[torch.Tensor] = None) -> None:
+                      cnt: Optional[torch.Tensor] = None, pool: Optional[dict] = None) -> None:
     if not 1 <= len(convs) <= 4:
         raise ValueError("conv_gemm_grouped: 1..4 convs")
     if variant not in GROUP_TILE:
@@ -264,15 +281,36 @@
                        Cin, OH, OW, Cout, k, k, 1, dil, ldo, co_off, Cout, ACT[c.get("act")],
                        _ptr(perm), Mp))
     _chk(order, torch.int32, "order")
-    if not getattr(order, "_ssa_checked", False):
+    npool, pool_t = 0, None
+    if pool is not None:
+        if variant not in GROUP_POOL_VARIANTS:
+            raise ValueError(f"conv_gemm_grouped: pool items need a variant in {GROUP_POOL_VARIANTS}")
+        npool, pHW, pC, pN = (pool[n] for n in ("B", "HW", "C", "N"))
+        if pC > 2048 or pN > 512 or pC % 8 or pN % 4 or npool < 1 or pHW < 1:
+            raise ValueError("conv_gemm_grouped: pool needs C <= 2048, C % 8, N <= 512, N % 4")
+        if not pool_item_fits(variant, pC, pN):
+            raise ValueError("conv_gemm_grouped: the pool work item does not fit this variant's LDS")
+        _chk(pool["x"], torch.bfloat16, "pool x", npool * pHW * pC)
+        _chk(pool["w1t"], torch.float32, "pool w1t", pC * pN)
+        _chk(pool["b1"], torch.float32, "pool b1", pN)
+        _chk(pool["w2t"], torch.float32, "pool w2t", pN * pN)
+        _chk(pool["img_bias"], torch.float32, "pool img_bias", npool * pN)
+        pool_t = (_ptr(pool["x"]), _ptr(pool["w1t"]), _ptr(pool["b1"]), _ptr(pool["w2t"]),
+                  _ptr(pool["img_bias"]), npool, pHW, pC, pN)
+    if not getattr(order, "_ssa_checked", None) == npool:
         oc = order.cpu().long()
+        isp = (oc >> 24) == POOL_GROUP
+        if sorted(oc[isp].tolist()) != [(POOL_GROUP << 24) | b for b in range(npool)]:
+            raise ValueError("conv_gemm_grouped: the order table must hold one pool item per image "
+                             "(and none without pool operands)")
+        oc = oc[~isp]
         g, t, sl = oc >> 24, oc & 0xFFFFF, (oc >> 20) & 15
         lim = torch.tensor(tiles)[g.clamp(0, len(tiles) - 1)]
         if (g < 0).any() or (g >= len(convs)).any() or (t >= lim).any() or (sl >= ks).any():
             raise ValueError("conv_gemm_grouped: order entry out of range")
         if oc.numel() != sum(tiles) * ks:
             raise ValueError("conv_gemm_grouped: the order table must list every tile's K slices once")
-        order._ssa_checked = True
+        order._ssa_checked = npool
     if ks > 1:
         c0 = convs[0]
         ldo, Mo = c0.get("ldo", c0["Cout"]), c0["B"] * c0["OH"] * c0["OW"]
@@ -290,7 +328,7 @@
             _chk(cnt, torch.int32, "cnt", 4 * max(tiles))
     _hip_mod().conv_gemm_grouped(groups, _ptr(order), order.numel(), variant, _stream(), int(ks),
                                  _ptr(part) if ks > 1 else 0, _ptr(cnt) if (ks > 1 and cnt is not None) else 0,
-                                 max(tiles))
+                                 max(tiles), pool_t)
     _dbg('conv_gemm_grouped')
     if ks > 1 and cnt is None:
         _hip_mod().stream_combine(_ptr(part), _ptr(bias_cat), 0, _ptr(c0["out"]), int(ks), Mo, ldo, _stream(),
```
